# yewsiang/Transferable3D

Measured on AMD Instinct MI355X. Metric: frustums/sec fwd+bwd, higher is better.
Workload: dtype f32

## Files before the change

### include/t3d.h

```cpp
#ifndef T3D_H_
#define T3D_H_

#include <stdint.h>

#ifdef __cplusplus
extern "C" {
#endif

#define T3D_OK 0
#define T3D_ERR_ARG (-1)
#define T3D_ERR_SHAPE (-2)
#define T3D_ERR_LAUNCH (-3)
#define T3D_ERR_ABI (-4)

#define T3D_ABI_VERSION 3
#define T3D_V2_SIZE_pointmlp_fwd_args 200
#define T3D_V2_SIZE_pointmlp_dgrad_args 168
#define T3D_V2_SIZE_pointmlp_wgrad_args 144
#define T3D_V2_SIZE_pointmlp_dgrad_gram_args 168
#define T3D_V2_SIZE_pointmlp_gram_args 96
#define T3D_V2_SIZE_seg_head_args 208
#define T3D_V2_SIZE_boxpc_rep_args 104

#define T3D_TILE_ROWS 128
// ... 622 lines not shown
  int len;
  const int32_t* members;
  const int32_t* offsets;
  int n_groups;
} t3d_semi_list;
typedef struct {
  uint32_t struct_size;
  int method;
  t3d_semi_list list3d;
  t3d_semi_list list2d;
  const int32_t* perm;
  int perm_len;
  int B;
  uint32_t seed;
  float equal_prob;
  const float* hyper;
  int32_t* sample;
  int32_t* is_data_2D;
} t3d_semi_sample_args;
#define T3D_V2_SIZE_semi_sample_args 136
int t3d_semi_sample(const t3d_semi_sample_args* args, t3d_stream_t stream);

#define T3D_NUM_CLASS 10
typedef struct {
  uint32_t struct_size;
  int F;
  const int32_t* cls;
  const uint8_t* member;
  const int32_t* class_mask;
  float keep_prob;
  float add_prob;
  uint32_t seed;
  int reserved;
  int32_t* ids;
  int32_t* members;
  int32_t* offsets;
  int32_t* present;
  int32_t* summary;
} t3d_label_subset_args;
#define T3D_V2_SIZE_label_subset_args 88
int t3d_label_subset(const t3d_label_subset_args* args, t3d_stream_t stream);

typedef struct {
  float* center;
  int32_t* orient_cls;
  float* orient_reg;
  const int32_t* dims_cls;
  float* dims_reg;
  float* y_box_iou;
  float* y_center_delta;
  float* y_dims_delta;
  float* y_orient_delta;
  float center_perturbation, size_perturbation, angle_perturbation;
  float fit_lo, fit_hi, nofit_lo, nofit_hi, proportion_fit;
  const float* fit_draw;
  const float* cand_draws;
  int max_rounds;
  uint32_t seed;
  const float* hyper;
  int B;
} t3d_boxpc_perturb_args;
int t3d_boxpc_perturb(const t3d_boxpc_perturb_args* args, t3d_stream_t stream);


typedef struct { int64_t slab_off; int64_t grad_off; int32_t numel; int32_t n_slabs; } t3d_slab_desc;
int t3d_reduce_slabs(const float* slab_base, float* grad_base, const t3d_slab_desc* table_dev,
                     int n_tensors, int max_numel, t3d_stream_t stream);
int t3d_pool_bwd_mid(const float* slab_base, float* grad_base, const t3d_slab_desc* table_dev, int n_tensors, int max_numel,
                     const t3d_pool_sparse_rows_args* sparse, t3d_stream_t stream);

typedef struct {
  float base_lr, lr_decay_rate, lr_decay_step;
  float bn_init_decay, bn_decay_rate, bn_decay_step, bn_decay_clip;
  float beta1, beta2;
  int batch_size;
  int step_offset;
} t3d_schedule;
int t3d_schedule_step(float* hyper, const t3d_schedule* s, t3d_stream_t stream);

int t3d_adam_tf_step(float* params, const float* grads, float* m, float* v, int64_t n,
                     const float* hyper, float beta1, float beta2, float eps, float grad_scale,
                     t3d_stream_t stream);

int t3d_split_x3(const float* src, void* planes, int64_t n, int64_t plane_stride, t3d_stream_t stream);

typedef struct {
  int64_t off;
  int32_t K, N;
  int32_t fwd, dgrad;
  int32_t blk0;
  int32_t reserved;
} t3d_x3_frag_entry;
int t3d_split_x3_frag(const float* params, void* planes_fwd, void* planes_dgrad, int64_t plane_stride, const t3d_x3_frag_entry* table,
                      int n_entries, int n_blocks, t3d_stream_t stream);

int t3d_momentum_step(float* params, const float* grads, float* accum, int64_t n, const float* hyper, float momentum,
                      float grad_scale, t3d_stream_t stream);

typedef struct {
  t3d_act_src a;
  const float* mask;
  float keep_prob;
  float* out;
  int M, K;
  int rows_per_frustum;
} t3d_act_dropout_args;
int t3d_act_dropout(const t3d_act_dropout_args* args, t3d_stream_t stream);

int t3d_cast_bf16(const float* src, void* dst, int64_t n, t3d_stream_t stream);

int t3d_dropout_mask(float* mask, int64_t n, float keep_prob, uint32_t seed, const float* hyper,
                     t3d_stream_t stream);

enum { T3D_SMALL_BN_BWD_FINALIZE = 1, T3D_SMALL_FC_BWD = 2, T3D_SMALL_FC_DINPUT = 3, T3D_SMALL_DY_COLSUM = 4,
       T3D_SMALL_BN_FWD_FINALIZE = 5, T3D_SMALL_FC_FWD = 6, T3D_SMALL_POOL_BWD_MID = 7 };
typedef struct {
  const float* slab_base;
  float* grad_base;
  const t3d_slab_desc* table_dev;
  int n_tensors, max_numel;
  t3d_pool_sparse_rows_args sparse;
} t3d_pool_bwd_mid_args;
typedef struct {
  int kind;
  int depends;
  union {
    t3d_bn_bwd_finalize_args bn_bwd;
    t3d_fc_bwd_args fc_bwd;
    t3d_fc_dinput_args fc_dinput;
    t3d_dy_colsum_args dy_colsum;
    t3d_bn_fwd_finalize_args bn_fwd;
    t3d_fc_fwd_args fc_fwd;
    t3d_pool_bwd_mid_args mid;
  } u;
} t3d_small_op;
int t3d_small_pair(const t3d_small_op* a, const t3d_small_op* b, t3d_stream_t stream);

#define T3D_RIDER_MAX_OPS 10
typedef struct {
  t3d_small_op ops[T3D_RIDER_MAX_OPS];
  int n_ops;
  int n_wg;
  int lds_bytes;
  unsigned* sync;
} t3d_rider_set;
int t3d_riders_plan(t3d_rider_set* riders);
int t3d_run_riders(const t3d_rider_set* riders, t3d_stream_t stream);
int t3d_pointmlp_fwd_r(const t3d_pointmlp_fwd_args* args, const t3d_rider_set* riders, t3d_stream_t stream);
int t3d_pointmlp_wgrad_r(const t3d_pointmlp_wgrad_args* args, const t3d_rider_set* riders, t3d_stream_t stream);
int t3d_pointmlp_bwd_r(const t3d_pointmlp_dgrad_args* dgrad, const t3d_pointmlp_wgrad_args* wgrad, const t3d_rider_set* riders,
                       t3d_stream_t stream);
int t3d_pool_bwd_stage1_r(const t3d_pointmlp_gram_args* gram, const t3d_act_colsum_args* colsum, const t3d_pool_bwd_prep_args* prep,
                          const t3d_rider_set* riders, t3d_stream_t stream);
int t3d_pool_bwd_stage2_r(const t3d_pool_wgrad_finish_args* finish, const t3d_pointmlp_dgrad_gram_args* dgrad,
                          const t3d_rider_set* riders, t3d_stream_t stream);
int t3d_pointmlp_fwd_hosts_riders(const t3d_pointmlp_fwd_args* args);
int t3d_pointmlp_wgrad_hosts_riders(const t3d_pointmlp_wgrad_args* args);
int t3d_pointmlp_bwd_hosts_riders(const t3d_pointmlp_dgrad_args* dgrad, const t3d_pointmlp_wgrad_args* wgrad);
int t3d_pool_bwd_stage1_hosts_riders(const t3d_pointmlp_gram_args* gram, const t3d_act_colsum_args* colsum, const t3d_pool_bwd_prep_args* prep);
int t3d_pool_bwd_stage2_hosts_riders(const t3d_pool_wgrad_finish_args* finish, const t3d_pointmlp_dgrad_gram_args* dgrad);

typedef struct {
  uint32_t struct_size;
  const double* points;
  const int64_t* scene_offsets;
  const double* rtilt;
  const double* K;
  const int32_t* scene_jobs;
  int n_scenes; int max_scene_points; int C_src; int C; int n_jobs; int num_points;
  const double* box2d;
  int perturb_box2d;
  const double* perturb_draws;
  const double* box3d;
  const int32_t* job_key;
  uint32_t seed;
  const int32_t* choice;
  const int64_t* mask_offsets;
// ... 80 lines not shown
```

### transferable3d_amd/abi.py

```python
import ctypes as C
import os

F = C.POINTER(C.c_float)
I = C.POINTER(C.c_int32)
D = C.POINTER(C.c_double)
L = C.POINTER(C.c_int64)
i32, f32 = C.c_int, C.c_float

TILE_ROWS = 128
F32, BF16 = 0, 1
DTYPE_BY_NAME = {'f32': F32, 'bf16': BF16}
ARITH_AUTO, ARITH_FP32_MFMA, ARITH_BF16X3, ARITH_BF16 = 0, 1, 2, 3
ARITH_BY_NAME = {'auto': ARITH_AUTO, 'fp32_mfma': ARITH_FP32_MFMA, 'bf16x3': ARITH_BF16X3}
ARITH_NAMES = {ARITH_FP32_MFMA: 'fp32_mfma', ARITH_BF16X3: 'bf16x3', ARITH_BF16: 'bf16'}
ABI_VERSION = 3
ERR_ABI = -4
ACT_NONE, ACT_RELU, ACT_LEAKY_RELU, ACT_TANH = 0, 1, 2, 3
ACT_BY_NAME = {None: ACT_NONE, 'relu': ACT_RELU, 'leaky_relu': ACT_LEAKY_RELU, 'tanh': ACT_TANH}


class Sized(C.Structure):

    def __init__(self, *args, **kw):
        super().__init__(C.sizeof(type(self)), *args, **kw)
# ... 129 lines not shown
    _fields_ = [('in_', F), ('ld_in', i32), ('K', i32), ('in2', F), ('ld_in2', i32), ('K2', i32), ('w', F), ('bias', F),
                ('gamma', F), ('beta', F), ('moving_mean', F), ('moving_var', F), ('decay', F), ('eps', f32),
                ('is_training', i32), ('unbiased_ema', i32), ('act', i32), ('leaky_alpha', f32), ('drop_mask', F),
                ('keep_prob', f32), ('add_in', F), ('ld_add', i32), ('add_n', i32), ('y', F), ('out', F),
                ('ld_out', i32), ('mean', F), ('invstd', F), ('B', i32), ('N', i32)]


class FcBwdArgs(C.Structure):
    _fields_ = [('dout', F), ('ld_dout', i32), ('dy_next', F), ('w_next', F), ('N_next', i32),
                ('in_', F), ('ld_in', i32), ('K', i32), ('in2', F), ('ld_in2', i32), ('K2', i32),
                ('y', F), ('out', F), ('ld_out', i32), ('gamma', F), ('beta', F), ('mean', F), ('invstd', F),
                ('bn_training', i32), ('act', i32), ('leaky_alpha', f32), ('drop_mask', F), ('keep_prob', f32),
                ('dy', F), ('dw', F), ('dbias', F), ('dgamma', F), ('dbeta', F), ('B', i32), ('N', i32)]


class FcDinputArgs(C.Structure):
    _fields_ = [('dy', F), ('N', i32), ('w', F), ('add_in', F), ('ld_add', i32), ('alpha', f32), ('din', F),
                ('ld_din', i32), ('B', i32), ('K', i32),
                ('bn_pooled', F), ('bn_ld_pooled', i32), ('bn_ysel', F), ('bn_dpool', F), ('bn_count', i32), ('bn_gamma', F), ('bn_mean', F),
                ('bn_invstd', F), ('bn_scale', F), ('bn_frozen', i32), ('bn_dgamma', F), ('bn_dbeta', F), ('bn_coef', F)]


class SegHeadArgs(Sized):
    _fields_ = [('struct_size', C.c_uint32), ('y', F), ('scale', F), ('shift', F), ('drop_mask', F), ('keep_prob', f32), ('w', F), ('bias', F),
                ('labels', I), ('is_data_2D', I), ('pc', F), ('ld_pc', i32), ('ce_weight', f32), ('logits', F),
                ('mask', F), ('part', F), ('dz', F), ('psum_dz', F), ('psum_dzy', F), ('dw_part', F),
                ('M', i32), ('K', i32), ('rows_per_frustum', i32), ('B', i32), ('drop_seed', C.c_uint32), ('drop_hyper', F),
                ('dtype', i32), ('dsoft', F), ('oracle_mask', I)]


SMALL_KIND = {'t3d_bn_bwd_finalize': 1, 't3d_fc_bwd': 2, 't3d_fc_dinput': 3, 't3d_dy_colsum': 4}
RIDER_KIND = dict(SMALL_KIND, t3d_bn_fwd_finalize=5, t3d_fc_fwd=6, t3d_pool_bwd_mid=7)
RIDER_FIELD = {1: 'bn_bwd', 2: 'fc_bwd', 3: 'fc_dinput', 4: 'dy_colsum', 5: 'bn_fwd', 6: 'fc_fwd', 7: 'mid'}
RIDER_WIDE = ('t3d_pool_bwd_mid',)


class WeakLossArgs(C.Structure):
    _fields_ = [('center', F), ('reg_dims', F), ('reg_theta', F), ('pc', F), ('ld_pc', i32), ('logits', F), ('Rtilt', F), ('K', F),
                ('rot_frust', F), ('box2D', F), ('img_dim', F), ('is_data_2D', I), ('w_reproj', f32), ('w_surface', f32),
                ('multiplier', f32), ('use_softmax_proj', i32), ('softmax_scale', f32), ('dilate', f32), ('clip_lower_b_loss', i32),
                ('clip_pred_box', i32), ('loss_mse', i32), ('train_box_reproj', i32 * 3), ('train_box_surface', i32 * 3),
                ('surface_margin', f32), ('surface_scale_dims', f32), ('surf_part', F), ('dsoft', F), ('reproj', F), ('surface', F),
                ('dbox7', F), ('total_losses', F), ('loss', F), ('B', i32), ('N', i32), ('one_hot', F), ('w_inactive', f32),
                ('inactive_margins', f32 * 10), ('inactive_train', i32 * 10), ('inactive', F)]


class ActDropoutArgs(C.Structure):
    _fields_ = [('a', ActSrc), ('mask', F), ('keep_prob', f32), ('out', F), ('M', i32), ('K', i32), ('rows_per_frustum', i32)]


class SegFinalizeArgs(C.Structure):
    _fields_ = [('part', F), ('dw_part', F), ('B', i32), ('tiles_per_frustum', i32), ('rows_per_frustum', i32),
                ('K', i32), ('mask_xyz_mean', F), ('seg_loss', F), ('dw', F), ('dbias', F), ('n_correct', F)]


class StrongWeights(C.Structure):
    _fields_ = [(n, f32) for n in ('center', 'orient_cls', 'orient_reg', 'dims_cls', 'dims_reg', 'tnet_center',
                                   'corner', 'box_multiplier', 'cross_entropy')]


class StrongLossArgs(C.Structure):
    _fields_ = [('box', F), ('ld_box', i32), ('stage1_center', F), ('seg_loss', F), ('y_center', F),
                ('y_orient_cls', I), ('y_orient_reg', F), ('y_dims_cls', I), ('y_dims_reg', F), ('is_data_2D', I),
                ('wts', StrongWeights), ('normalize_by_3d_count', i32), ('dbox', F), ('dstage1', F), ('terms', F),
                ('total_losses', F), ('loss', F), ('center', F), ('reg_dims', F), ('reg_theta', F), ('iou2d', F), ('iou3d', F), ('B', i32)]


class X3FragEntry(C.Structure):
    _fields_ = [('off', C.c_int64), ('K', C.c_int32), ('N', C.c_int32), ('fwd', C.c_int32), ('dgrad', C.c_int32), ('blk0', C.c_int32), ('reserved', C.c_int32)]


def x3_frag_table(entries):
    import numpy as np
    rec = np.zeros(len(entries), dtype=np.dtype([('off', '<i8'), ('K', '<i4'), ('N', '<i4'), ('fwd', '<i4'), ('dgrad', '<i4'), ('blk0', '<i4'), ('reserved', '<i4')]))
    blk = 0
    for i, (off, K, N) in enumerate(entries):
        rec[i] = (off, K, N, 1, 1, blk, 0)
        blk += (K * N // 8 + 255) // 256
    return rec.view(np.uint8).copy(), blk


class SlabDesc(C.Structure):
    _fields_ = [('slab_off', C.c_int64), ('grad_off', C.c_int64), ('numel', C.c_int32), ('n_slabs', C.c_int32)]


class Schedule(C.Structure):
    _fields_ = [('base_lr', f32), ('lr_decay_rate', f32), ('lr_decay_step', f32), ('bn_init_decay', f32),
                ('bn_decay_rate', f32), ('bn_decay_step', f32), ('bn_decay_clip', f32), ('beta1', f32), ('beta2', f32),
                ('batch_size', i32), ('step_offset', i32)]


class BoxPcRepArgs(Sized):
    _fields_ = [('struct_size', C.c_uint32), ('pc', F), ('ld_pc', i32), ('C', i32), ('center', F), ('dims', F), ('theta', F), ('y_dims_cls', I),
                ('y_orient_cls', I), ('rep', F), ('ld_rep', i32), ('box_out', F), ('M', i32), ('rows_per_frustum', i32), ('rowmask', F)]


class BoxPcRepBArgs(C.Structure):
    _fields_ = [('center', F), ('dims', F), ('theta', F), ('y_dims_cls', I), ('y_orient_cls', I), ('box_out', F), ('pc', F), ('ld_pc', i32),
                ('C', i32), ('rowmask', F), ('pc_out', F), ('ld_out', i32), ('B', i32), ('rows_per_frustum', i32)]


class BoxPcRepBwdArgs(C.Structure):
    _fields_ = [('pc', F), ('ld_pc', i32), ('box', F), ('drep', F), ('ld_drep', i32), ('coff', i32), ('dbox', F),
                ('B', i32), ('rows_per_frustum', i32)]


class BoxPcLossArgs(C.Structure):
    _fields_ = [('out', F), ('y_box_iou', F), ('y_center_delta', F), ('y_dims_delta', F), ('y_orient_delta', F),
                ('fit_bound', f32), ('w_cls', f32), ('w_delta', f32), ('w_center', f32), ('w_size', f32), ('w_angle', f32),
                ('weigh_by_cls_conf', i32), ('weigh_by_cls_gt', i32), ('dout', F), ('terms', F), ('loss', F), ('B', i32),
                ('weigh_pred_by_cls_conf', i32), ('grad_cls_via_delta', i32), ('delta_loss_mse', i32)]


class BoxRefineStepBwdArgs(C.Structure):
    _fields_ = [('out9', F), ('dbox_rep', F), ('carry', F), ('tot_out', F), ('dout9', F), ('weigh_by_conf', i32),
                ('grad_via_conf', i32), ('B', i32)]


class Box2dFeatsArgs(C.Structure):
    _fields_ = [('one_hot', F), ('n_oh', i32), ('box2D', F), ('img_dim', F), ('out', F), ('B', i32)]


class DgradNarrowArgs(C.Structure):
    _fields_ = [('dy', DySrc), ('w', F), ('k0', i32), ('kn', i32), ('out', F), ('ld_out', i32), ('M', i32), ('N', i32)]


class SemiFinalLossArgs(C.Structure):
    _fields_ = [('strong_loss', F), ('reg_dims', F), ('one_hot', F), ('is_data_2D', I), ('out9', F),
                ('train_classes', C.c_int32 * 10), ('w_weak', f32), ('w_fit', f32), ('fit_only_2d', i32), ('d_dims', F),
                ('dout9', F), ('fit_prob', F), ('terms', F), ('loss', F), ('B', i32)]


class AnchorRegBwdArgs(C.Structure):
    _fields_ = [('box', F), ('ld_box', i32), ('dbox7', F), ('d_dims', F), ('dbox', F), ('dstage1', F), ('B', i32)]


class FrustumExtractArgs(Sized):
    _fields_ = [('struct_size', C.c_uint32), ('points', D), ('scene_offsets', L), ('rtilt', D), ('K', D), ('scene_jobs', I),
                ('n_scenes', i32), ('max_scene_points', i32), ('C_src', i32), ('C', i32), ('n_jobs', i32), ('num_points', i32),
                ('box2d', D), ('perturb_box2d', i32), ('perturb_draws', D), ('box3d', D), ('job_key', I), ('seed', C.c_uint32),
                ('choice', I), ('mask_offsets', L), ('masks', C.POINTER(C.c_uint64)), ('seg_prefix', I), ('box2d_out', D),
                ('frustum_angle', D), ('n_in_box', I), ('count', I), ('index', I), ('out_points', D), ('label', I)]


U8 = C.POINTER(C.c_uint8)


class SunrgbdEvalArgs(Sized):
    _fields_ = [('struct_size', C.c_uint32), ('P', i32), ('G', i32), ('det_centroid', D), ('det_basis', D), ('det_coeffs', D),
                ('det_confidence', D), ('det_image', I), ('gt_centroid', D), ('gt_basis', D), ('gt_coeffs', D), ('gt_image', I),
                ('gt_difficult', U8), ('n_images', i32), ('image_ids', I), ('image_gt_offsets', I), ('image_gt', I),
                ('threshold', C.c_double), ('workspace', C.c_void_p), ('workspace_bytes', C.c_uint64), ('order', I), ('max_overlap', D),
                ('gt_idx', I), ('is_tp', U8), ('is_fp', U8), ('gt_assignment', I), ('is_missed', U8), ('precision', D), ('recall', D),
                ('ap', D), ('overlap_offsets', L), ('overlaps', D), ('overlap_gt', I)]


SEMI_BATCH, SEMI_ALTERNATE_BATCH, SEMI_MIXED_BATCH = 0, 1, 2
SEMI_METHODS = {'BATCH': SEMI_BATCH, 'ALTERNATE_BATCH': SEMI_ALTERNATE_BATCH, 'MIXED_BATCH': SEMI_MIXED_BATCH}
SEMI_SAMPLE_MAX_B = 256


class SemiList(C.Structure):
    _fields_ = [('ids', I), ('len', i32), ('members', I), ('offsets', I), ('n_groups', i32)]


class SemiSampleArgs(Sized):
# ... 25 lines not shown
    _fields_ = [('slab_base', F), ('grad_base', F), ('table_dev', C.POINTER(SlabDesc)), ('n_tensors', i32), ('max_numel', i32),
                ('sparse', PoolSparseRowsArgs)]


class SmallOpU(C.Union):
    _fields_ = [('bn_bwd', BnBwdFinalizeArgs), ('fc_bwd', FcBwdArgs), ('fc_dinput', FcDinputArgs), ('dy_colsum', DyColsumArgs),
                ('bn_fwd', BnFwdFinalizeArgs), ('fc_fwd', FcFwdArgs), ('mid', PoolBwdMidArgs)]


class SmallOp(C.Structure):
    _fields_ = [('kind', i32), ('depends', i32), ('u', SmallOpU)]


RIDER_MAX_OPS = 10


class RiderSet(C.Structure):
    _fields_ = [('ops', SmallOp * RIDER_MAX_OPS), ('n_ops', i32), ('n_wg', i32), ('lds_bytes', i32), ('sync', C.POINTER(C.c_uint32))]


ENTRY_POINTS = {
    't3d_abi_version': [],
    't3d_gemm_arithmetic': [i32, i32, i32, i32, i32],
    't3d_source_hash': [C.c_char_p, C.c_int],
    't3d_pointmlp_fwd': [C.POINTER(PointMlpFwdArgs), VP],
    't3d_bn_fwd_finalize': [C.POINTER(BnFwdFinalizeArgs), VP],
    't3d_pool_finalize': [C.POINTER(PoolFinalizeArgs), VP],
    't3d_pointmlp_dgrad': [C.POINTER(PointMlpDgradArgs), VP],
    't3d_pointmlp_wgrad': [C.POINTER(PointMlpWgradArgs), VP],
    't3d_pointmlp_bwd': [C.POINTER(PointMlpDgradArgs), C.POINTER(PointMlpWgradArgs), VP],
    't3d_wgrad_plan': [i32, i32, i32, C.POINTER(i32), C.POINTER(i32), C.POINTER(i32)],
    't3d_bwd_plan': [i32, i32, i32, i32, C.POINTER(i32), C.POINTER(i32)],
    't3d_weak_loss': [C.POINTER(WeakLossArgs), VP],
    't3d_small_pair': [C.POINTER(SmallOp), C.POINTER(SmallOp), VP],
    't3d_riders_plan': [C.POINTER(RiderSet)],
    't3d_run_riders': [C.POINTER(RiderSet), VP],
    't3d_pointmlp_fwd_r': [C.POINTER(PointMlpFwdArgs), C.POINTER(RiderSet), VP],
    't3d_pointmlp_wgrad_r': [C.POINTER(PointMlpWgradArgs), C.POINTER(RiderSet), VP],
    't3d_pointmlp_bwd_r': [C.POINTER(PointMlpDgradArgs), C.POINTER(PointMlpWgradArgs), C.POINTER(RiderSet), VP],
    't3d_pool_bwd_stage1_r': [C.POINTER(PointMlpGramArgs), C.POINTER(ActColsumArgs), C.POINTER(PoolBwdPrepArgs), C.POINTER(RiderSet), VP],
    't3d_pool_bwd_stage2_r': [C.POINTER(PoolWgradFinishArgs), C.POINTER(PointMlpDgradGramArgs), C.POINTER(RiderSet), VP],
    't3d_pointmlp_fwd_hosts_riders': [C.POINTER(PointMlpFwdArgs)],
    't3d_pointmlp_wgrad_hosts_riders': [C.POINTER(PointMlpWgradArgs)],
    't3d_pointmlp_bwd_hosts_riders': [C.POINTER(PointMlpDgradArgs), C.POINTER(PointMlpWgradArgs)],
    't3d_pool_bwd_stage1_hosts_riders': [C.POINTER(PointMlpGramArgs), C.POINTER(ActColsumArgs), C.POINTER(PoolBwdPrepArgs)],
    't3d_pool_bwd_stage2_hosts_riders': [C.POINTER(PoolWgradFinishArgs), C.POINTER(PointMlpDgradGramArgs)],
    't3d_gram_plan': [i32, i32, i32, C.POINTER(i32), C.POINTER(i32)],
    't3d_bn_bwd_finalize': [C.POINTER(BnBwdFinalizeArgs), VP],
    't3d_dy_colsum': [C.POINTER(DyColsumArgs), VP],
    't3d_pool_bwd_prep': [C.POINTER(PoolBwdPrepArgs), VP],
    't3d_pool_sparse_rows': [C.POINTER(PoolSparseRowsArgs), VP],
    't3d_pointmlp_dgrad_gram': [C.POINTER(PointMlpDgradGramArgs), VP],
    't3d_pointmlp_gram': [C.POINTER(PointMlpGramArgs), VP],
    't3d_act_colsum': [C.POINTER(ActColsumArgs), VP],
    't3d_pool_wgrad_finish': [C.POINTER(PoolWgradFinishArgs), VP],
    't3d_batch_assemble': [C.POINTER(BatchAssembleArgs), VP],
    't3d_box_refine_step': [C.POINTER(BoxRefineStepArgs), VP],
    't3d_box_refine_step_bwd': [C.POINTER(BoxRefineStepBwdArgs), VP],
    't3d_boxpc_perturb': [C.POINTER(BoxPcPerturbArgs), VP],
    't3d_sample_equal_classes': [C.POINTER(SampleEqualClassesArgs), VP],
    't3d_box3d_iou': [C.POINTER(Box3dIouArgs), VP],
    't3d_box3d_iou_corners': [C.POINTER(Box3dIouCornersArgs), VP],
    't3d_box_head_iou': [C.POINTER(BoxHeadIouArgs), VP],
    't3d_box2d_feats': [C.POINTER(Box2dFeatsArgs), VP],
    't3d_pool_bwd_stage1': [C.POINTER(PointMlpGramArgs), C.POINTER(ActColsumArgs), C.POINTER(PoolBwdPrepArgs), VP],
    't3d_pool_bwd_mid': [F, F, C.POINTER(SlabDesc), i32, i32, C.POINTER(PoolSparseRowsArgs), VP],
    't3d_pool_bwd_stage2': [C.POINTER(PoolWgradFinishArgs), C.POINTER(PointMlpDgradGramArgs), VP],
    't3d_fc_fwd': [C.POINTER(FcFwdArgs), VP],
    't3d_fc_bwd': [C.POINTER(FcBwdArgs), VP],
    't3d_fc_dinput': [C.POINTER(FcDinputArgs), VP],
    't3d_seg_head': [C.POINTER(SegHeadArgs), VP],
    't3d_seg_finalize': [C.POINTER(SegFinalizeArgs), VP],
    't3d_act_dropout': [C.POINTER(ActDropoutArgs), VP],
    't3d_strong_loss': [C.POINTER(StrongLossArgs), VP],
    't3d_boxpc_rep': [C.POINTER(BoxPcRepArgs), VP],
    't3d_boxpc_rep_b': [C.POINTER(BoxPcRepBArgs), VP],
    't3d_boxpc_rep_bwd': [C.POINTER(BoxPcRepBwdArgs), VP],
    't3d_boxpc_loss': [C.POINTER(BoxPcLossArgs), VP],
    't3d_pointmlp_dgrad_narrow': [C.POINTER(DgradNarrowArgs), VP],
    't3d_semi_final_loss': [C.POINTER(SemiFinalLossArgs), VP],
    't3d_anchor_reg_bwd': [C.POINTER(AnchorRegBwdArgs), VP],
    't3d_reduce_slabs': [F, F, C.POINTER(SlabDesc), i32, i32, VP],
    't3d_schedule_step': [F, C.POINTER(Schedule), VP],
    't3d_adam_tf_step': [F, F, F, F, C.c_int64, F, f32, f32, f32, f32, VP],
    't3d_momentum_step': [F, F, F, C.c_int64, F, f32, f32, VP],
    't3d_split_x3': [F, VP, C.c_int64, C.c_int64, VP],
    't3d_split_x3_frag': [F, VP, VP, C.c_int64, VP, i32, i32, VP],
    't3d_dropout_mask': [F, C.c_int64, f32, C.c_uint32, F, VP],
    't3d_cast_bf16': [F, VP, C.c_int64, VP],
    't3d_frustum_extract': [C.POINTER(FrustumExtractArgs), VP],
    't3d_sunrgbd_eval': [C.POINTER(SunrgbdEvalArgs), VP],
    't3d_detect_decode': [C.POINTER(DetectDecodeArgs), VP],
    't3d_semi_sample': [C.POINTER(SemiSampleArgs), VP],
    't3d_label_subset': [C.POINTER(LabelSubsetArgs), VP],
}

LIB_PATH = os.path.join(os.path.dirname(os.path.abspath(__file__)), 'libt3d.so')
ERRORS = {-1: 'T3D_ERR_ARG', -2: 'T3D_ERR_SHAPE', -3: 'T3D_ERR_LAUNCH'}


class T3DError(RuntimeError):
    pass


def source_hash_of(lib):
    buf = C.create_string_buffer(64)
    check(lib.t3d_source_hash(buf, 64), 't3d_source_hash')
    return buf.value.decode()


def load(path=None):
    import torch
    variant = path or os.environ.get('T3D_LIB')
    path = variant or LIB_PATH
    if not os.path.exists(path):
        raise T3DError('HIP library %s not built: run `python -m transferable3d_amd.build` (no CPU fallback exists)' % path)
    lib = C.CDLL(path)
    for name, argtypes in ENTRY_POINTS.items():
        fn = getattr(lib, name, None)
        if fn is None:
            raise T3DError('%s does not export %s' % (path, name))
        fn.argtypes = argtypes
        fn.restype = C.c_int
    if lib.t3d_abi_version() != ABI_VERSION:
        raise T3DError('%s speaks ABI version %d, this host side version %d (include/t3d.h): rebuild it' % (path, lib.t3d_abi_version(), ABI_VERSION))
    from .build import CSRC, lib_source_hash
    if not variant and os.path.isdir(CSRC) and os.environ.get('T3D_ALLOW_STALE_LIB', '0') != '1':
        built, src = source_hash_of(lib), lib_source_hash()
        if built != src:
            raise T3DError('%s was built from other sources (library %s, csrc/ + include/t3d.h %s): run '
                           '`python -m transferable3d_amd.build`' % (path, built, src))
    return lib


def fptr(t):
    return C.cast(C.c_void_p(0 if t is None else t.data_ptr()), F)


def iptr(t):
    return C.cast(C.c_void_p(0 if t is None else t.data_ptr()), I)


def u8ptr(t):
    return C.cast(C.c_void_p(0 if t is None else t.data_ptr()), U8)


def check(rc, what):
    if rc != 0:
        raise T3DError('%s failed: %s' % (what, ERRORS.get(rc, rc)))
```

### transferable3d_amd/csrc/bn_dev.h

```cpp
#pragma once
#include "common.h"
#include <math.h>

namespace {

constexpr int FC_CH = 16, FC_GR = 16, FC_GR_BIG = 64, FC_CH_WIDE = 4, FC_GR_WIDE = 256, FC_WIDE_MAX_N = 128;

template <int NQ, int GR = FC_GR, int U = 16>
__device__ __forceinline__ void tile_sums(const float* const (&src)[NQ], int n_tiles, int N, int c, int grp, bool ok,
                                          double (&acc)[NQ]) {
#pragma unroll
  for (int q = 0; q < NQ; ++q) acc[q] = 0.0;
  if (!ok) return;
  for (int t0 = grp; t0 < n_tiles; t0 += U * GR) {
    float v[NQ][U];
#pragma unroll
    for (int q = 0; q < NQ; ++q)
#pragma unroll
      for (int u = 0; u < U; ++u) {
        const int t = t0 + u * GR;
        const float x = src[q][(size_t)min(t, n_tiles - 1) * N + c];
        v[q][u] = t < n_tiles ? x : 0.f;
      }
#pragma unroll
// ... 98 lines not shown
      const bool take = (t0 + u < tiles_per_frustum) && a[u] >= 0 && (arg < 0 || (use_max ? v[u] > best : v[u] < best));
      best = take ? v[u] : best;
      arg = take ? a[u] : arg;
    }
  }
  float out = 0.f;
  if (arg >= 0) out = fmaxf(fmaf(best, sc, sh), 0.f);
  const bool live = out > 0.f;
  const size_t i = (size_t)b * N + c;
  pooled[(size_t)b * ld_pooled + c] = out;
  argidx[i] = live ? arg : -1;
  ysel[i] = live ? best : 0.f;
}
__device__ __forceinline__ void pool_pick(const t3d_bn_fwd_finalize_args& p, int b, int c, float sc, float sh) {
  pool_pick_impl(p.pool_pmax, p.pool_pmin, p.pool_pamax, p.pool_pamin, p.pool_tiles_per_frustum, p.N, b, c, sc, sh, p.pooled,
                 p.ld_pooled, p.argidx, p.ysel);
}

template <int GR, int CH = FC_CH>
__device__ __forceinline__ void bn_fwd_finalize_body(const t3d_bn_fwd_finalize_args& p, double (*red)[CH], float* s_scsh, const int bid) {
  const int cl = threadIdx.x & (CH - 1), grp = threadIdx.x / CH;
  const int c = bid * CH + cl;
  const bool ok = c < p.N;
  if (p.is_training) {
    const int cc = ok ? c : 0;
    const float gam = p.gamma[cc], bet = p.beta[cc], mm = p.moving_mean[cc], mv = p.moving_var[cc], dec = p.decay[0];
    const float* const src[2] = {p.psum, p.psumsq};
    double acc[2];
    tile_sums<2, GR, (GR > 64 ? 8 : 16)>(src, p.n_tiles, p.N, c, grp, ok, acc);
    const double s = group_reduce<GR, CH>(acc[0], red, grp, cl);
    const double ss = group_reduce<GR, CH>(acc[1], red, grp, cl);
    if (grp == 0 && ok) {
      const double n = (double)p.count;
      const double mean = s / n;
      double var = ss / n - mean * mean;
      if (var < 0.0) var = 0.0;
      const double invstd = 1.0 / sqrt(var + (double)p.eps);
      const double sc = (double)gam * invstd;
      p.scale[c] = (float)sc;
      p.shift[c] = (float)((double)bet - mean * sc);
      p.mean[c] = (float)mean;
      p.invstd[c] = (float)invstd;
      const double d = (double)dec;
      const double var_ema = p.unbiased_ema ? var * (n / (n > 1.0 ? n - 1.0 : 1.0)) : var;
      p.moving_mean[c] = (float)((double)mm * d + mean * (1.0 - d));
      p.moving_var[c] = (float)((double)mv * d + var_ema * (1.0 - d));
    }
  } else if (grp == 0 && ok) {
    const double invstd = 1.0 / sqrt((double)p.moving_var[c] + (double)p.eps);
    const double sc = (double)p.gamma[c] * invstd;
    p.scale[c] = (float)sc;
    p.shift[c] = (float)((double)p.beta[c] - (double)p.moving_mean[c] * sc);
    p.mean[c] = p.moving_mean[c];
    p.invstd[c] = (float)invstd;
  }
  if (p.pool_pmax != nullptr) {
    float* s_sc = s_scsh;
    float* s_sh = s_scsh + CH;
    __syncthreads();
    if (grp == 0 && ok) { s_sc[cl] = p.scale[c]; s_sh[cl] = p.shift[c]; }
    __syncthreads();
    if (ok) {
      const float sc = s_sc[cl], sh = s_sh[cl];
      for (int b = grp; b < p.pool_B; b += GR) pool_pick(p, b, c, sc, sh);
    }
  }
}

__device__ __forceinline__ void dy_colsum_body(const t3d_dy_colsum_args& p, const int bid, const int tid) {
  const int i = bid * 256 + tid;
  if (tid >= 256 || i >= p.B * p.N) return;
  const int b = i / p.N, c = i % p.N;
  double sdz = 0.0, sy = 0.0;
  for (int t = 0; t < p.tiles_per_frustum; ++t) {
    const size_t o = (size_t)(b * p.tiles_per_frustum + t) * p.N + c;
    sdz += (double)p.psum_dz[o];
    sy += (double)p.psum_y[o];
  }
  const double v = (double)p.coef[c] * sdz + (double)p.coef[p.N + c] * sy +
                   (double)p.coef[2 * p.N + c] * (double)p.rows_per_frustum;
  p.out[i] = (float)((double)p.alpha * v);
}

__device__ __forceinline__ void reduce_slabs_body(const float* __restrict__ slab_base, float* __restrict__ grad_base,
                                                  const t3d_slab_desc* __restrict__ table, float4 (*part)[32], int bx, int by,
                                                  int gx) {
  const t3d_slab_desc d = table[by];
  const bool vec = ((d.slab_off | d.grad_off | (int64_t)d.numel) & 3) == 0;
  const int n4 = vec ? (d.numel >> 2) : 0;
  const int el = threadIdx.x & 31, grp = threadIdx.x >> 5;
  for (int e0 = bx * 32; e0 < n4; e0 += gx * 32) {
    const int e = e0 + el;
    float4 a0 = make_float4(0.f, 0.f, 0.f, 0.f), a1 = a0, a2 = a0, a3 = a0;
    if (e < n4) {
      const float4* s = reinterpret_cast<const float4*>(slab_base + d.slab_off) + e;
      int k = grp;
      for (; k + 56 < d.n_slabs; k += 64) {
        float4 v[8];
#pragma unroll
        for (int u = 0; u < 8; ++u) v[u] = s[(size_t)(k + 8 * u) * n4];
#pragma unroll
        for (int u = 0; u < 8; u += 4) {
          a0.x += v[u].x; a0.y += v[u].y; a0.z += v[u].z; a0.w += v[u].w;
          a1.x += v[u + 1].x; a1.y += v[u + 1].y; a1.z += v[u + 1].z; a1.w += v[u + 1].w;
          a2.x += v[u + 2].x; a2.y += v[u + 2].y; a2.z += v[u + 2].z; a2.w += v[u + 2].w;
          a3.x += v[u + 3].x; a3.y += v[u + 3].y; a3.z += v[u + 3].z; a3.w += v[u + 3].w;
        }
      }
      for (; k + 24 < d.n_slabs; k += 32) {
        const float4 v0 = s[(size_t)(k + 0) * n4], v1 = s[(size_t)(k + 8) * n4], v2 = s[(size_t)(k + 16) * n4],
                     v3 = s[(size_t)(k + 24) * n4];
        a0.x += v0.x; a0.y += v0.y; a0.z += v0.z; a0.w += v0.w;
        a1.x += v1.x; a1.y += v1.y; a1.z += v1.z; a1.w += v1.w;
        a2.x += v2.x; a2.y += v2.y; a2.z += v2.z; a2.w += v2.w;
        a3.x += v3.x; a3.y += v3.y; a3.z += v3.z; a3.w += v3.w;
      }
      for (; k < d.n_slabs; k += 8) {
        const float4 v = s[(size_t)k * n4];
        a0.x += v.x; a0.y += v.y; a0.z += v.z; a0.w += v.w;
      }
    }
    float4 r;
    r.x = (a0.x + a1.x) + (a2.x + a3.x); r.y = (a0.y + a1.y) + (a2.y + a3.y);
    r.z = (a0.z + a1.z) + (a2.z + a3.z); r.w = (a0.w + a1.w) + (a2.w + a3.w);
    part[grp][el] = r;
    __syncthreads();
    if (grp == 0 && e < n4) {
      float4 t = part[0][el];
#pragma unroll
      for (int g = 1; g < 8; ++g) {
        const float4 u = part[g][el];
        t.x += u.x; t.y += u.y; t.z += u.z; t.w += u.w;
      }
      reinterpret_cast<float4*>(grad_base + d.grad_off)[e] = t;
    }
    __syncthreads();
  }
  if (!vec) {
    for (int e = bx * blockDim.x + threadIdx.x; e < d.numel; e += gx * blockDim.x) {
      float acc = 0.f;
      for (int k = 0; k < d.n_slabs; ++k) acc += slab_base[d.slab_off + (size_t)k * d.numel + e];
      grad_base[d.grad_off + e] = acc;
    }
  }
}


}
```

### transferable3d_amd/csrc/bn_optim.hip

```cpp
#include "common.h"
#include "poolbwd_dev.h"
#include "bn_dev.h"

namespace {

template <int GR, int CH = FC_CH>
__global__ __launch_bounds__(GR * CH) void k_bn_fwd_finalize(const t3d_bn_fwd_finalize_args p) {
  __shared__ double red[GR][CH];
  __shared__ float s_scsh[2 * CH];
  bn_fwd_finalize_body<GR, CH>(p, red, s_scsh, blockIdx.x);
}

__global__ __launch_bounds__(256) void k_pool_finalize(const t3d_pool_finalize_args p) {
  const int i = blockIdx.x * blockDim.x + threadIdx.x;
  if (i >= p.B * p.N) return;
  const int b = i / p.N, c = i % p.N;
  pool_pick_impl(p.pmax, p.pmin, p.pamax, p.pamin, p.tiles_per_frustum, p.N, b, c, p.scale[c], p.shift[c], p.pooled, p.ld_pooled,
                 p.argidx, p.ysel);
}

template <int GR, int CH = FC_CH>
__global__ __launch_bounds__(GR * CH) void k_bn_bwd_finalize(const t3d_bn_bwd_finalize_args p) {
  __shared__ double red[GR][CH];
  bn_bwd_finalize_body<GR, CH>(p, red, blockIdx.x, threadIdx.x);
}

__global__ __launch_bounds__(256) void k_dy_colsum(const t3d_dy_colsum_args p) { dy_colsum_body(p, blockIdx.x, threadIdx.x); }

__global__ __launch_bounds__(256) void k_reduce_slabs(const float* __restrict__ slab_base, float* __restrict__ grad_base,
                                                      const t3d_slab_desc* __restrict__ table) {
  __shared__ float4 part[8][32];
  reduce_slabs_body(slab_base, grad_base, table, part, blockIdx.x, blockIdx.y, gridDim.x);
}

__global__ __launch_bounds__(256) void k_pool_bwd_mid(const float* __restrict__ slab_base, float* __restrict__ grad_base,
                                                      const t3d_slab_desc* __restrict__ table, const int gx, const int n_reduce,
                                                      const t3d_pool_sparse_rows_args sp) {
  extern __shared__ __attribute__((aligned(16))) float smem[];
  const int b = blockIdx.x;
  if (b < n_reduce) {
    reduce_slabs_body(slab_base, grad_base, table, reinterpret_cast<float4(*)[32]>(smem), b % gx, b / gx, gx);
  } else {
    const int r = b - n_reduce, tiles = sp.B * sp.rows_per_frustum / 128;
    pool_sparse_rows_body(sp, smem, r % tiles, r / tiles);
  }
}

__global__ __launch_bounds__(64) void k_schedule_step(float* hyper, const t3d_schedule s) {
  if (blockIdx.x != 0) return;
  const int lane = threadIdx.x;
  const double step = (double)hyper[0] + (double)s.step_offset;
  const double seen = step * (double)s.batch_size;
  const double t = step + 1.0;
  const double base = lane == 0 ? (double)s.lr_decay_rate : lane == 1 ? (double)s.bn_decay_rate : lane == 2 ? (double)s.beta2 : (double)s.beta1;
  const double expo = lane == 0 ? floor(seen / (double)s.lr_decay_step) : lane == 1 ? floor(seen / (double)s.bn_decay_step) : t;
  const double pw = lane < 4 ? pow(base, expo) : 0.0;
  const double p_lr = __shfl(pw, 0), p_bn = __shfl(pw, 1), p_b2 = __shfl(pw, 2), p_b1 = __shfl(pw, 3);
  if (lane != 0) return;
  const double lr = (double)s.base_lr * p_lr;
  const double bnm = (double)s.bn_init_decay * p_bn;
  const double bnd = fmin((double)s.bn_decay_clip, 1.0 - bnm);
  const double lr_t = lr * sqrt(1.0 - p_b2) / (1.0 - p_b1);
  hyper[1] = (float)lr;
  hyper[2] = (float)bnd;
  hyper[3] = (float)lr_t;
  hyper[0] = (float)t;
}

__global__ __launch_bounds__(256) void k_adam_tf(float* __restrict__ w, const float* __restrict__ g, float* __restrict__ m,
                                                 float* __restrict__ v, int64_t n, const float* __restrict__ hyper,
                                                 float b1, float b2, float eps, float gscale) {
  const float lr_t = hyper[3];
  for (int64_t i = (int64_t)blockIdx.x * blockDim.x + threadIdx.x; i < n; i += (int64_t)gridDim.x * blockDim.x) {
    const float gi = g[i] * gscale;
    const float mi = b1 * m[i] + (1.f - b1) * gi;
    const float vi = b2 * v[i] + (1.f - b2) * gi * gi;
    m[i] = mi;
    v[i] = vi;
    w[i] -= lr_t * mi / (sqrtf(vi) + eps);
  }
}

__global__ __launch_bounds__(256) void k_momentum_tf(float* __restrict__ w, const float* __restrict__ g, float* __restrict__ acc,
                                                     int64_t n, const float* __restrict__ hyper, float momentum, float gscale) {
  const float lr = hyper[1];
  for (int64_t i = (int64_t)blockIdx.x * blockDim.x + threadIdx.x; i < n; i += (int64_t)gridDim.x * blockDim.x) {
    const float a = fmaf(momentum, acc[i], g[i] * gscale);
    acc[i] = a;
    w[i] -= lr * a;
  }
}

__device__ __forceinline__ uint32_t mix_u32(uint64_t x) {
  x ^= x >> 33; x *= 0xff51afd7ed558ccdULL;
  x ^= x >> 33; x *= 0xc4ceb9fe1a85ec53ULL;
  x ^= x >> 33;
  return (uint32_t)(x >> 16);
}
__global__ __launch_bounds__(256) void k_dropout_mask(float* __restrict__ mask, int64_t n, float keep, uint32_t seed,
                                                      const float* __restrict__ hyper) {
  const uint64_t step = (uint64_t)hyper[0];
  const uint64_t key = ((uint64_t)seed << 32) ^ (step * 0x9E3779B97F4A7C15ULL);
  for (int64_t i = (int64_t)blockIdx.x * blockDim.x + threadIdx.x; i < n; i += (int64_t)gridDim.x * blockDim.x) {
    const uint32_t r = mix_u32(key + (uint64_t)i * 0xD6E8FEB86659FD93ULL);
    const float u = (float)(r >> 8) * (1.0f / 16777216.0f);
    mask[i] = u < keep ? 1.f : 0.f;
  }
}

}

extern "C" int t3d_abi_version(void) { return T3D_ABI_VERSION; }

static int fin_big_tiles() {
  static const int v = []() { const char* e = getenv("T3D_FIN_BIG"); const int x = e ? atoi(e) : 512; return x > 0 ? x : (1 << 30); }();
  return v;
}

static int fin_wide_tiles() {
  static const int v = []() { const char* e = getenv("T3D_FIN_WIDE"); const int x = e ? atoi(e) : 1024; return x > 0 ? x : (1 << 30); }();
  return v;
}

extern "C" int t3d_bn_fwd_finalize(const t3d_bn_fwd_finalize_args* a, t3d_stream_t stream) {
  if (!a || !a->gamma || !a->beta || !a->moving_mean || !a->moving_var || !a->scale || !a->shift || !a->mean ||
      !a->invstd)
    return T3D_ERR_ARG;
  if (a->is_training && (!a->psum || !a->psumsq || !a->decay || a->count <= 0)) return T3D_ERR_ARG;
  if (a->is_training && a->n_tiles >= fin_wide_tiles() && a->N <= FC_WIDE_MAX_N)
    T3D_LAUNCH((k_bn_fwd_finalize<FC_GR_WIDE, FC_CH_WIDE>), dim3((a->N + FC_CH_WIDE - 1) / FC_CH_WIDE), dim3(FC_GR_WIDE * FC_CH_WIDE), 0,
               static_cast<hipStream_t>(stream), *a);
  else if (a->is_training && a->n_tiles > fin_big_tiles())
    T3D_LAUNCH(k_bn_fwd_finalize<FC_GR_BIG>, dim3((a->N + FC_CH - 1) / FC_CH), dim3(FC_GR_BIG * FC_CH), 0, static_cast<hipStream_t>(stream), *a);
  else
    T3D_LAUNCH(k_bn_fwd_finalize<FC_GR>, dim3((a->N + FC_CH - 1) / FC_CH), dim3(FC_GR * FC_CH), 0, static_cast<hipStream_t>(stream), *a);
  T3D_CHECK_LAUNCH();
  return T3D_OK;
}

extern "C" int t3d_pool_finalize(const t3d_pool_finalize_args* a, t3d_stream_t stream) {
  if (!a || !a->scale || !a->shift || !a->pmax || !a->pmin || !a->pamax || !a->pamin || !a->pooled || !a->argidx ||
      !a->ysel)
    return T3D_ERR_ARG;
  T3D_LAUNCH(k_pool_finalize, dim3((a->B * a->N + 255) / 256), dim3(256), 0, static_cast<hipStream_t>(stream),
                     *a);
  T3D_CHECK_LAUNCH();
  return T3D_OK;
}

extern "C" int t3d_bn_bwd_finalize(const t3d_bn_bwd_finalize_args* a, t3d_stream_t stream) {
  if (!a || !a->coef) return T3D_ERR_ARG;
  if (a->psum_dz == nullptr && (!a->dpool_in || !a->pooled || !a->ysel || !a->dpool)) return T3D_ERR_ARG;
  if (a->psum_dz != nullptr && !a->psum_dzy) return T3D_ERR_ARG;
  if (a->frozen ? !a->scale : (!a->gamma || !a->mean || !a->invstd)) return T3D_ERR_ARG;
  if (a->psum_dz != nullptr && a->n_tiles >= fin_wide_tiles() && a->N <= FC_WIDE_MAX_N)
    T3D_LAUNCH((k_bn_bwd_finalize<FC_GR_WIDE, FC_CH_WIDE>), dim3((a->N + FC_CH_WIDE - 1) / FC_CH_WIDE), dim3(FC_GR_WIDE * FC_CH_WIDE), 0,
               static_cast<hipStream_t>(stream), *a);
  else if (a->psum_dz != nullptr && a->n_tiles > fin_big_tiles())
    T3D_LAUNCH(k_bn_bwd_finalize<FC_GR_BIG>, dim3((a->N + FC_CH - 1) / FC_CH), dim3(FC_GR_BIG * FC_CH), 0, static_cast<hipStream_t>(stream), *a);
  else
    T3D_LAUNCH(k_bn_bwd_finalize<FC_GR>, dim3((a->N + FC_CH - 1) / FC_CH), dim3(FC_GR * FC_CH), 0, static_cast<hipStream_t>(stream), *a);
  T3D_CHECK_LAUNCH();
  return T3D_OK;
}

extern "C" int t3d_dy_colsum(const t3d_dy_colsum_args* a, t3d_stream_t stream) {
  if (!a || !a->psum_dz || !a->psum_y || !a->coef || !a->out) return T3D_ERR_ARG;
  T3D_LAUNCH(k_dy_colsum, dim3((a->B * a->N + 255) / 256), dim3(256), 0, static_cast<hipStream_t>(stream), *a);
  T3D_CHECK_LAUNCH();
  return T3D_OK;
}

extern "C" int t3d_reduce_slabs(const float* slab_base, float* grad_base, const t3d_slab_desc* table_dev, int n_tensors,
                                int max_numel, t3d_stream_t stream) {
  if (!slab_base || !grad_base || !table_dev || n_tensors <= 0) return T3D_ERR_ARG;
  int gx = (max_numel / 4 + 31) / 32;
  if (gx > 256) gx = 256;
  if (gx < 1) gx = 1;
  T3D_LAUNCH(k_reduce_slabs, dim3(gx, n_tensors), dim3(256), 0, static_cast<hipStream_t>(stream), slab_base,
                     grad_base, table_dev);
  T3D_CHECK_LAUNCH();
  return T3D_OK;
}

extern "C" int t3d_schedule_step(float* hyper, const t3d_schedule* s, t3d_stream_t stream) {
  if (!hyper || !s) return T3D_ERR_ARG;
  T3D_LAUNCH(k_schedule_step, dim3(1), dim3(64), 0, static_cast<hipStream_t>(stream), hyper, *s);
  T3D_CHECK_LAUNCH();
  return T3D_OK;
}

extern "C" int t3d_adam_tf_step(float* params, const float* grads, float* m, float* v, int64_t n, const float* hyper,
                                float beta1, float beta2, float eps, float grad_scale, t3d_stream_t stream) {
  if (!params || !grads || !m || !v || !hyper || n <= 0) return T3D_ERR_ARG;
  int64_t blocks = (n + 255) / 256;
  if (blocks > 2048) blocks = 2048;
  T3D_LAUNCH(k_adam_tf, dim3((unsigned)blocks), dim3(256), 0, static_cast<hipStream_t>(stream), params, grads, m,
                     v, n, hyper, beta1, beta2, eps, grad_scale);
  T3D_CHECK_LAUNCH();
  return T3D_OK;
}

extern "C" int t3d_momentum_step(float* params, const float* grads, float* accum, int64_t n, const float* hyper, float momentum,
                                 float grad_scale, t3d_stream_t stream) {
  if (!params || !grads || !accum || !hyper || n <= 0) return T3D_ERR_ARG;
  int64_t blocks = (n + 255) / 256;
  if (blocks > 2048) blocks = 2048;
  T3D_LAUNCH(k_momentum_tf, dim3((unsigned)blocks), dim3(256), 0, static_cast<hipStream_t>(stream), params, grads, accum, n, hyper,
             momentum, grad_scale);
  T3D_CHECK_LAUNCH();
  return T3D_OK;
}

__global__ __launch_bounds__(256) void k_cast_bf16(const float* __restrict__ src, bf16_t* __restrict__ dst, int64_t n) {
  const int64_t stride = (int64_t)gridDim.x * 256 * 8;
  for (int64_t i = ((int64_t)blockIdx.x * 256 + threadIdx.x) * 8; i < n; i += stride) {
    if (i + 8 <= n) {
      const float4 a = *reinterpret_cast<const float4*>(src + i), b = *reinterpret_cast<const float4*>(src + i + 4);
      const bf16x8 h = {(bf16_t)a.x, (bf16_t)a.y, (bf16_t)a.z, (bf16_t)a.w, (bf16_t)b.x, (bf16_t)b.y, (bf16_t)b.z, (bf16_t)b.w};
      *reinterpret_cast<bf16x8*>(dst + i) = h;
    } else {
      for (int64_t j = i; j < n; ++j) dst[j] = (bf16_t)src[j];
    }
  }
}

extern "C" int t3d_cast_bf16(const float* src, void* dst, int64_t n, t3d_stream_t stream) {
  if (!src || !dst || n <= 0 || (reinterpret_cast<uintptr_t>(src) & 15) || (reinterpret_cast<uintptr_t>(dst) & 15)) return T3D_ERR_ARG;
  int64_t blocks = (n + 2047) / 2048;
  if (blocks > 2048) blocks = 2048;
  T3D_LAUNCH(k_cast_bf16, dim3((unsigned)blocks), dim3(256), 0, static_cast<hipStream_t>(stream), src, static_cast<bf16_t*>(dst), n);
  T3D_CHECK_LAUNCH();
  return T3D_OK;
}

extern "C" int t3d_dropout_mask(float* mask, int64_t n, float keep_prob, uint32_t seed, const float* hyper,
                                t3d_stream_t stream) {
  if (!mask || !hyper || n <= 0) return T3D_ERR_ARG;
  int64_t blocks = (n + 255) / 256;
  if (blocks > 4096) blocks = 4096;
  T3D_LAUNCH(k_dropout_mask, dim3((unsigned)blocks), dim3(256), 0, static_cast<hipStream_t>(stream), mask, n,
                     keep_prob, seed, hyper);
  T3D_CHECK_LAUNCH();
  return T3D_OK;
}

extern "C" int t3d_pool_bwd_mid(const float* slab_base, float* grad_base, const t3d_slab_desc* table_dev, int n_tensors,
                                int max_numel, const t3d_pool_sparse_rows_args* a, t3d_stream_t stream) {
  if (!slab_base || !grad_base || !table_dev || n_tensors <= 0) return T3D_ERR_ARG;
  const int rc = check_sparse_rows(a);
  if (rc != T3D_OK) return rc;
  int gx = (max_numel / 4 + 31) / 32;
  if (gx > 256) gx = 256;
  if (gx < 1) gx = 1;
  const int n_reduce = gx * n_tensors;
  const long M = (long)a->B * a->rows_per_frustum;
  const int n_sparse = (int)(M / 128) * (a->K / SR_KC);
  const size_t lds = sparse_rows_lds(a->N);
  static size_t allowed = 0;
  if (lds > 64 * 1024 && lds > allowed) {
    (void)hipFuncSetAttribute(reinterpret_cast<const void*>(k_pool_bwd_mid), hipFuncAttributeMaxDynamicSharedMemorySize, (int)lds);
    allowed = lds;
  }
  T3D_LAUNCH(k_pool_bwd_mid, dim3(n_reduce + n_sparse), dim3(256), lds, static_cast<hipStream_t>(stream), slab_base, grad_base,
             table_dev, gx, n_reduce, *a);
  T3D_CHECK_LAUNCH();
  return T3D_OK;
}
```

### transferable3d_amd/csrc/pointmlp.hip

```cpp
#include "common.h"
#include "poolbwd_dev.h"
#include "rider_dev.h"

#include <cstdlib>
#include <mutex>
#include <type_traits>
#include <utility>
#include <unordered_map>

namespace {

constexpr int BK = 32;
constexpr int MIN_WAVES_PER_EU = 2;
constexpr int LDR = BK + 4;
constexpr int NT = 256;

__device__ __forceinline__ float4 f4zero() { return make_float4(0.f, 0.f, 0.f, 0.f); }

__device__ __forceinline__ unsigned keep_bits32(const float* __restrict__ rowmask, int base) {
  float4 m[8];
#pragma unroll
  for (int q = 0; q < 8; ++q) m[q] = *reinterpret_cast<const float4*>(rowmask + base + (q >> 2) * 32 + (q & 3) * 8);
  unsigned bits = 0u;
#pragma unroll
// ... 1675 lines not shown
          for (int r = 0; r < 16; ++r) {
            const float v = SY ? Elem<bf16_t>::rnd(acc[tm][tn][r] + add) : acc[tm][tn][r] + add;
            if constexpr (SY) ytile[(wm * 64 + 4 * h + tm * 32 + (r & 3) + 8 * (r >> 2)) * YLD + wn * (BN / 2) + tn * 32 + l31] = (bf16_t)v;
            s_ += v;
            ss = fmaf(v, v, ss);
            if constexpr (PL) {
              const bool keep = (keepbits >> (tm * 16 + r)) & 1u;
              const int rin = rin_base + tm * 32 + (r & 3) + 8 * (r >> 2);
              const bool up = keep & (v > mx), dn = keep & (v < mn);
              mx = up ? v : mx;
              ax = up ? rin : ax;
              mn = dn ? v : mn;
              an = dn ? rin : an;
            }
          }
        }
        s_ += __shfl_xor(s_, 32, 64);
        ss += __shfl_xor(ss, 32, 64);
        if constexpr (PL) {
          const float omx = __shfl_xor(mx, 32, 64), omn = __shfl_xor(mn, 32, 64);
          const int oax = __shfl_xor(ax, 32, 64), oan = __shfl_xor(an, 32, 64);
          if (oax >= 0 && (omx > mx || ax < 0 || (omx == mx && oax < ax))) { mx = omx; ax = oax; }
          if (oan >= 0 && (omn < mn || an < 0 || (omn == mn && oan < an))) { mn = omn; an = oan; }
        }
        csum[tn] = s_; csq[tn] = ss; cmax[tn] = mx; cmin[tn] = mn; amax[tn] = ax; amin[tn] = an;
      }
    };
    if (store_y) { if (pool) epi(std::true_type{}, std::true_type{}); else epi(std::true_type{}, std::false_type{}); }
    else { if (pool) epi(std::false_type{}, std::true_type{}); else epi(std::false_type{}, std::false_type{}); }
    if (h == 0) {
#pragma unroll
      for (int tn = 0; tn < TN; ++tn) {
        const int c = wn * (BN / 2) + tn * 32 + l31;
        red[(0 * 2 + wm) * BN + c] = csum[tn];
        red[(1 * 2 + wm) * BN + c] = csq[tn];
        if (pool) {
          red[(2 * 2 + wm) * BN + c] = cmax[tn];
          red[(3 * 2 + wm) * BN + c] = cmin[tn];
          reinterpret_cast<int*>(red)[(4 * 2 + wm) * BN + c] = amax[tn];
          reinterpret_cast<int*>(red)[(5 * 2 + wm) * BN + c] = amin[tn];
        }
      }
    }
    if (tr_first && nt == 0) T3D_TRACE_MARK8(4);
    __syncthreads();
    if (tid < BN) {
      const int c = tid;
      const size_t o = (size_t)tile_m * p.N + col0 + c;
      p.psum[o] = red[(0 * 2 + 0) * BN + c] + red[(0 * 2 + 1) * BN + c];
      p.psumsq[o] = red[(1 * 2 + 0) * BN + c] + red[(1 * 2 + 1) * BN + c];
      if (pool) {
        float mx = red[(2 * 2 + 0) * BN + c], mn = red[(3 * 2 + 0) * BN + c];
        int ax = reinterpret_cast<int*>(red)[(4 * 2 + 0) * BN + c], an = reinterpret_cast<int*>(red)[(5 * 2 + 0) * BN + c];
        const float mx1 = red[(2 * 2 + 1) * BN + c], mn1 = red[(3 * 2 + 1) * BN + c];
        const int ax1 = reinterpret_cast<int*>(red)[(4 * 2 + 1) * BN + c], an1 = reinterpret_cast<int*>(red)[(5 * 2 + 1) * BN + c];
        if (ax1 >= 0 && (ax < 0 || mx1 > mx)) { mx = mx1; ax = ax1; }
        if (an1 >= 0 && (an < 0 || mn1 < mn)) { mn = mn1; an = an1; }
        p.pmax[o] = mx; p.pmin[o] = mn; p.pamax[o] = ax; p.pamin[o] = an;
      }
    }
    if (tr_first && nt == 0) T3D_TRACE_MARK8(5);
    if constexpr (LAST) {
      fetch_w0(0, (tile_nx * 128) / p.rows_per_frustum);
      if constexpr (PREF) fetch_panel_coefs();
    } else {
      fetch_w0(col0 + BN, b);
    }
    if (store_y) {
#pragma unroll
      for (int i = 0; i < 128 * CPR / NT; ++i) {
        const int c = tid + NT * i, row = c / CPR, ch = c % CPR;
        *reinterpret_cast<bf16x8*>(yg + (size_t)(row0 + row) * p.N + col0 + ch * 8) = *reinterpret_cast<const bf16x8*>(ytile + row * YLD + ch * 8);
      }
    }
    if (tr_first && nt == 0) T3D_TRACE_MARK8(6);
  };
#pragma unroll 1
  for (int nt = 0; nt < n_tiles - 1; ++nt) col_tile(nt, std::false_type{});
  col_tile(n_tiles - 1, std::true_type{});
 }
  T3D_TRACE_MARK8(7);
}

template <int N, class YT = bf16_t>
__global__ __launch_bounds__(NT) void k_pointmlp_fwd_tinyk(const t3d_pointmlp_fwd_args p) {
  constexpr bool H = Elem<YT>::BF16;
  constexpr int CPR = N / 8, RPP = NT / CPR, NP = 128 / RPP;
  __shared__ float red[2][RPP][N];
  const int tid = threadIdx.x, ch = tid % CPR, r0 = tid / CPR;
  const int tile = blockIdx.x, row0 = tile * 128, b = row0 / p.rows_per_frustum;
  float w[4][8], add[8];
#pragma unroll
  for (int k = 0; k < 4; ++k) {
    if (H) {
      const bf16x8 v = *reinterpret_cast<const bf16x8*>(reinterpret_cast<const bf16_t*>(p.w) + (size_t)min(k, p.K - 1) * p.N + ch * 8);
#pragma unroll
      for (int e = 0; e < 8; ++e) w[k][e] = k < p.K ? (float)v[e] : 0.f;
    } else {
      const float4 v0 = *reinterpret_cast<const float4*>(p.w + (size_t)min(k, p.K - 1) * p.N + ch * 8);
      const float4 v1 = *reinterpret_cast<const float4*>(p.w + (size_t)min(k, p.K - 1) * p.N + ch * 8 + 4);
      const float v[8] = {v0.x, v0.y, v0.z, v0.w, v1.x, v1.y, v1.z, v1.w};
#pragma unroll
      for (int e = 0; e < 8; ++e) w[k][e] = k < p.K ? v[e] : 0.f;
    }
  }
#pragma unroll
  for (int e = 0; e < 8; ++e) add[e] = p.bias ? p.bias[ch * 8 + e] : 0.f;
  float sc[4] = {1.f, 1.f, 1.f, 1.f}, sh[4] = {0.f, 0.f, 0.f, 0.f}, sub[4] = {0.f, 0.f, 0.f, 0.f};
  if (p.a.scale != nullptr) {
    const float4 a = *reinterpret_cast<const float4*>(p.a.scale), c = *reinterpret_cast<const float4*>(p.a.shift);
    sc[0] = a.x; sc[1] = a.y; sc[2] = a.z; sc[3] = a.w; sh[0] = c.x; sh[1] = c.y; sh[2] = c.z; sh[3] = c.w;
  }
  if (p.a.sub != nullptr) {
#pragma unroll
    for (int k = 0; k < 4; ++k) sub[k] = p.a.sub[(size_t)b * p.a.sub_ld + min(k, p.K - 1)];
  }
  const float floor_ = p.a.relu ? 0.f : -INFINITY;
  float s1[8], s2[8];
#pragma unroll
  for (int e = 0; e < 8; ++e) { s1[e] = 0.f; s2[e] = 0.f; }
  float4 xs[NP];
#pragma unroll
  for (int i = 0; i < NP; ++i) xs[i] = *reinterpret_cast<const float4*>(p.a.x + (size_t)(row0 + r0 + RPP * i) * p.a.ldx + p.a.coff);
#pragma unroll
  for (int i = 0; i < NP; ++i) {
    const float xv[4] = {xs[i].x, xs[i].y, xs[i].z, xs[i].w};
    float a[4];
#pragma unroll
    for (int k = 0; k < 4; ++k) {
      const float t = fmaxf(fmaf(xv[k], sc[k], sh[k]), floor_) - sub[k];
      a[k] = k < p.K ? Elem<YT>::rnd(t) : 0.f;
    }
    float o[8];
#pragma unroll
    for (int e = 0; e < 8; ++e) {
      float acc = a[0] * w[0][e];
      acc = fmaf(a[1], w[1][e], acc);
      acc = fmaf(a[2], w[2][e], acc);
      acc = fmaf(a[3], w[3][e], acc);
      const float v = Elem<YT>::rnd(acc + add[e]);
      o[e] = v;
      s1[e] += v;
      s2[e] = fmaf(v, v, s2[e]);
    }
    const size_t off = (size_t)(row0 + r0 + RPP * i) * p.N + ch * 8;
    if (H) {
      bf16x8 ob;
#pragma unroll
      for (int e = 0; e < 8; ++e) ob[e] = (bf16_t)o[e];
      *reinterpret_cast<bf16x8*>(reinterpret_cast<bf16_t*>(p.y) + off) = ob;
    } else {
      *reinterpret_cast<float4*>(p.y + off) = make_float4(o[0], o[1], o[2], o[3]);
      *reinterpret_cast<float4*>(p.y + off + 4) = make_float4(o[4], o[5], o[6], o[7]);
    }
  }
#pragma unroll
  for (int e = 0; e < 8; ++e) { red[0][r0][ch * 8 + e] = s1[e]; red[1][r0][ch * 8 + e] = s2[e]; }
  __syncthreads();
  if (tid < N) {
    float t1 = 0.f, t2 = 0.f;
#pragma unroll
    for (int r = 0; r < RPP; ++r) { t1 += red[0][r][tid]; t2 += red[1][r][tid]; }
    p.psum[(size_t)tile * p.N + tid] = t1;
    p.psumsq[(size_t)tile * p.N + tid] = t2;
  }
}

struct DgradEpilogue {
  const float* add_in;
  const int32_t* add_live;
  const float* colconst;
  const float* prev_y;
  const float* prev_scale;
  const float* prev_shift;
  float* out;
  float* psum_dz;
  float* psum_dzy;
  int K;
};

template <int BN, int TM, int TN, int ADD, bool MASK>
__device__ __forceinline__ void dgrad_epilogue_body(const DgradEpilogue& p, f32x16 (&acc)[TM][TN], float* red, int tid,
                                                    int row0, int col0, int tile_m) {
  const int lane = tid & 63, wid = tid >> 6, wm = wid >> 1, wn = wid & 1;
  const int l31 = lane & 31, h = lane >> 5;
  const bool stats = MASK && p.psum_dz != nullptr;
  const unsigned K = (unsigned)p.K;
  float cs1[TN], cs2[TN];
  unsigned live = 0u;
  if (ADD == 2) {
    int4 fl[TM][4];
#pragma unroll
    for (int tm = 0; tm < TM; ++tm)
#pragma unroll
      for (int j = 0; j < 4; ++j) fl[tm][j] = *reinterpret_cast<const int4*>(p.add_live + row0 + wm * 64 + 4 * h + tm * 32 + 8 * j);
#pragma unroll
    for (int tm = 0; tm < TM; ++tm)
#pragma unroll
      for (int j = 0; j < 4; ++j) {
        const int4 f = fl[tm][j];
        live |= (unsigned)((f.x != 0) | ((f.y != 0) << 1) | ((f.z != 0) << 2) | ((f.w != 0) << 3)) << (tm * 16 + 4 * j);
      }
  }
#pragma unroll
  for (int tn = 0; tn < TN; ++tn) {
    const int col = col0 + wn * (BN / 2) + tn * 32 + l31;
    const float psc = MASK ? p.prev_scale[col] : 0.f, psh = MASK ? p.prev_shift[col] : 0.f;
    const float cc = p.colconst ? p.colconst[col] : 0.f;
    unsigned boff0 = ((unsigned)(row0 + wm * 64 + 4 * h) * K + (unsigned)col) * 4u;
    asm volatile("" : "+v"(boff0));
    const unsigned k4 = K * 4u;
    const char* const pyb = reinterpret_cast<const char*>(p.prev_y);
    const char* const adb = reinterpret_cast<const char*>(p.add_in);
    char* const outb = reinterpret_cast<char*>(p.out);
    float s1 = 0.f, s2 = 0.f;
#pragma unroll
    for (int tm = 0; tm < TM; ++tm) {
      constexpr int EB = 8;
#pragma unroll
      for (int r0 = 0; r0 < 16; r0 += EB) {
        float yp[EB], ad[EB];
#pragma unroll
        for (int e = 0; e < EB; ++e) {
          const int r = r0 + e;
          const unsigned o = boff0 + (unsigned)(tm * 32 + (r & 3) + 8 * (r >> 2)) * k4;
          yp[e] = MASK ? *reinterpret_cast<const float*>(pyb + o) : 0.f;
          if (ADD == 2) ad[e] = ((live >> (tm * 16 + r)) & 1u) ? *reinterpret_cast<const float*>(adb + o) : 0.f;
          else ad[e] = ADD ? *reinterpret_cast<const float*>(adb + o) : 0.f;
        }
#pragma unroll
        for (int e = 0; e < EB; ++e) {
          const int r = r0 + e;
          const unsigned o = boff0 + (unsigned)(tm * 32 + (r & 3) + 8 * (r >> 2)) * k4;
          float v = acc[tm][tn][r] + cc + ad[e];
          if (MASK) {
            if (!(fmaf(yp[e], psc, psh) > 0.f)) v = 0.f;
            s1 += v;
            s2 = fmaf(v, yp[e], s2);
          }
          *reinterpret_cast<float*>(outb + o) = v;
        }
      }
    }
    s1 += __shfl_xor(s1, 32, 64);
    s2 += __shfl_xor(s2, 32, 64);
    cs1[tn] = s1; cs2[tn] = s2;
  }
  if (stats) {
// ... 1460 lines not shown
  static std::unordered_map<const void*, size_t> done;
  std::lock_guard<std::mutex> lock(mu);
  size_t& cur = done[kernel];
  if (cur >= lds_bytes) return;
  (void)hipFuncSetAttribute(kernel, hipFuncAttributeMaxDynamicSharedMemorySize, (int)lds_bytes);
  cur = lds_bytes;
}

template <class Args>
void launch_lds(void (*kernel)(const Args), dim3 grid, size_t lds_bytes, hipStream_t s, const Args& a) {
  allow_lds(reinterpret_cast<const void*>(kernel), lds_bytes);
  T3D_LAUNCH(kernel, grid, dim3(NT), lds_bytes, s, a);
}
template <class Args>
void launch_lds_r(void (*kernel)(const Args, const t3d_rider_set), dim3 grid, size_t lds_bytes, hipStream_t s, const Args& a,
                  const t3d_rider_set& r) {
  allow_lds(reinterpret_cast<const void*>(kernel), lds_bytes);
  T3D_LAUNCH(kernel, grid, dim3(NT), lds_bytes, s, a, r);
}
template <class Args>
void launch_lds1(void (*kernel)(const Args), dim3 grid, size_t lds_bytes, hipStream_t s, const Args& a) {
  allow_lds(reinterpret_cast<const void*>(kernel), lds_bytes);
  T3D_LAUNCH(kernel, grid, dim3(NT1), lds_bytes, s, a);
}
constexpr size_t lds_fwd(int bn) { return 2 * (size_t)(128 * LDR + BK * bn) * sizeof(float); }
constexpr size_t lds_dgrad(int bn) { return 2 * (size_t)(128 * LDR + bn * LDR) * sizeof(float); }
constexpr size_t lds_wgrad(int bmk, int bn) { return 2 * (size_t)BK * (bmk + bn) * sizeof(float); }
constexpr size_t lds_epi(int bn) { return (size_t)12 * bn * sizeof(float) + (size_t)128 * (bn + 8) * 2; }
constexpr size_t lds_min(size_t b, int bn) { return b > lds_epi(bn) ? b : lds_epi(bn); }
constexpr size_t lds_fwd_h(int bn) { return lds_min(2 * (size_t)(128 * LDRH + BKH * (bn + 32)) * 2, bn); }
constexpr size_t lds_dgram_h(int bn) { return lds_fwd_h(bn) > (size_t)12 * bn * 4 + 2 * (size_t)128 * (bn + 8) * 2 ? lds_fwd_h(bn) : (size_t)12 * bn * 4 + 2 * (size_t)128 * (bn + 8) * 2; }
constexpr size_t lds_epi2(int bn) { return (size_t)12 * bn * sizeof(float) + 2 * (size_t)128 * (bn + 8) * 2; }
constexpr size_t lds_max(size_t a, size_t b) { return a > b ? a : b; }
constexpr size_t lds_dgrad_h(int bn) { return lds_max(2 * (size_t)(128 * LDRH + bn * LDRH) * 2, lds_epi2(bn)); }
constexpr size_t lds_wgrad_h(int bmk, int bn) { return 2 * (size_t)BKH * (bmk + 32 + bn + 32) * 2; }
constexpr size_t lds_x3_r(int dim) { return (size_t)3 * dim * LDRX * 2; }
constexpr size_t lds_x3_c(int dim) { return (size_t)3 * BKX * (dim + LDCX_PAD) * 2; }
constexpr size_t lds_fwd_x3(int bn) { return lds_max(2 * (lds_x3_r(128) + lds_x3_c(bn)), (size_t)12 * bn * sizeof(float)); }
constexpr size_t lds_dgrad_x3(int bn) { return lds_max(2 * (lds_x3_r(128) + lds_x3_r(bn)), (size_t)12 * bn * sizeof(float)); }
constexpr size_t lds_wgrad_x3(int bmk, int bn) { return 2 * (lds_x3_c(bmk) + lds_x3_c(bn)); }
constexpr size_t lds_bwd1f(int k, int n) { return (size_t)(64 * ((n + 4) + 3 * (k + 4)) + 2 * 2 * 2 * k + 3 * n + 2 * k) * 4; }
constexpr size_t lds_bwd1(int k, int n, int bm) { return (size_t)bm * (n + k + 2 * (k + 8)) * 2 + (size_t)2 * 2 * 4 * k * 4; }

bool dtype_ok(int dt) { return dt == T3D_F32 || dt == T3D_BF16; }
bool x3_on(int arith) {
  if (arith == T3D_ARITH_FP32_MFMA) return false;
  if (arith == T3D_ARITH_BF16X3) return true;
  const char* e = getenv("T3D_X3");
  return e ? atoi(e) != 0 : true;
}
long x3_min_kn(int arith) { const char* e = arith == T3D_ARITH_AUTO ? getenv("T3D_X3_MINKN") : nullptr; return e ? atol(e) : 1L; }
long x3_min_kn_bwd(int arith) { const char* e = arith == T3D_ARITH_AUTO ? getenv("T3D_X3_MINKN_BWD") : nullptr; return e ? atol(e) : x3_min_kn(arith); }
bool x3_layer(int arith, int K, int N) { return x3_on(arith) && (long)K * N >= x3_min_kn(arith) && K <= 4096 && N <= 4096; }
bool x3_bwd_narrow() { const char* e = getenv("T3D_X3_BWD_NARROW"); return e ? atoi(e) != 0 : true; }
bool x3_layer_bwd(int arith, int K, int N) {
  return x3_on(arith) && (long)K * N >= x3_min_kn_bwd(arith) && (N <= 4 * K || K >= 128 || x3_bwd_narrow()) && K <= 4096 && N <= 4096;
}
bool act_ok(const t3d_act_src& a, int K) {
  return a.x != nullptr && (a.ldx % 4) == 0 && (a.coff % 4) == 0 && a.coff + (K + 3) / 4 * 4 <= a.ldx &&
         (a.scale == nullptr || a.shift != nullptr) && dtype_ok(a.dtype) && !(a.dtype == T3D_BF16 && a.sub != nullptr) &&
         !(a.dtype == T3D_BF16 && ((a.ldx | a.coff) & 7));
}
bool dy_ok(const t3d_dy_src& d) {
  return d.y != nullptr && d.coef != nullptr && (d.dz != nullptr || (d.argidx != nullptr && d.dpool != nullptr)) && dtype_ok(d.dtype) &&
         !(d.dtype == T3D_BF16 && d.dz == nullptr);
}

bool riders_ok(const t3d_rider_set* r) {
  return r->sync != nullptr && r->n_ops > 0 && r->n_ops <= T3D_RIDER_MAX_OPS && r->n_wg > 0 && r->n_wg <= (r->n_ops == 1 ? RIDER_MAX_WG_WIDE : RIDER_MAX_WG) && r->lds_bytes >= 0;
}
size_t lds_with(size_t lds, const t3d_rider_set* r) { return r && (size_t)r->lds_bytes > lds ? (size_t)r->lds_bytes : lds; }

}

int t3d_x3_fwd(const t3d_pointmlp_fwd_args* a, const t3d_rider_set* r, hipStream_t s);
int t3d_x3_bwd(const t3d_pointmlp_dgrad_args* d, const t3d_pointmlp_wgrad_args* w, const t3d_rider_set* r, int tk, int tn, bool wide,
               int n_w, int n_d, hipStream_t s);
int t3d_x3_stage1(const t3d_pointmlp_gram_args* g, const t3d_act_colsum_args* c, const t3d_pool_bwd_prep_args* q, const t3d_rider_set* r,
                  int gt, int n_gram, int n_colsum, int n_prep, size_t lds_other, hipStream_t s);
int t3d_x3_stage2(const t3d_pool_wgrad_finish_args* f, const t3d_pointmlp_dgrad_gram_args* d, const t3d_rider_set* r, bool wide,
                  int n_finish, int n_d, size_t lds_other, hipStream_t s);
int t3d_x3_split(const float* src, void* planes, int64_t n, int64_t plane_stride, hipStream_t s);
int t3d_x3_split_frag(const float* params, void* pf, void* pd, int64_t stride, const t3d_x3_frag_entry* tab, int n, int n_blocks, hipStream_t s);
int t3d_x3_dgrad(const t3d_pointmlp_dgrad_args* a, bool wide, hipStream_t s);
int t3d_x3_wgrad(const t3d_pointmlp_wgrad_args* a, int tk, int tn, int n_blocks, hipStream_t s);
int t3d_x3_gram(const t3d_pointmlp_gram_args* a, int tk, int n_blocks, hipStream_t s);
int t3d_x3_dgrad_gram(const t3d_pointmlp_dgrad_gram_args* a, bool wide, hipStream_t s);

#ifdef T3D_X3_TU
namespace {
__global__ __launch_bounds__(256) void k_split_x3(const float* __restrict__ src, bf16_t* __restrict__ planes, long n, long stride) {
  const long step = (long)gridDim.x * 256 * 4;
  for (long i = ((long)blockIdx.x * 256 + threadIdx.x) * 4; i < n; i += step) {
    if (i + 4 <= n) {
      bf16x4 h, m, l;
      split3(*reinterpret_cast<const float4*>(src + i), h, m, l);
      *reinterpret_cast<bf16x4*>(planes + i) = h;
      *reinterpret_cast<bf16x4*>(planes + stride + i) = m;
      *reinterpret_cast<bf16x4*>(planes + 2 * stride + i) = l;
    } else {
      for (long j = i; j < n; ++j) {
        bf16x4 h, m, l;
        split3(make_float4(src[j], 0.f, 0.f, 0.f), h, m, l);
        planes[j] = h[0]; planes[stride + j] = m[0]; planes[2 * stride + j] = l[0];
      }
    }
  }
}
}
namespace {
__global__ __launch_bounds__(256) void k_split_x3_frag(const float* __restrict__ params, bf16_t* __restrict__ pf, bf16_t* __restrict__ pd, long stride,
                                                       const t3d_x3_frag_entry* __restrict__ tab, int n) {
  int e = 0;
  while (e + 1 < n && (int)blockIdx.x >= tab[e + 1].blk0) ++e;
  const t3d_x3_frag_entry en = tab[e];
  const float* w = params + en.off;
  const long nfr = (long)en.K * en.N / 8;
  const long f = (long)((int)blockIdx.x - en.blk0) * 256 + threadIdx.x;
  if (f >= nfr) return;
  const int lane = (int)(f & 63);
  const long q = f >> 6;
  float4 v0, v1, u0, u1;
  if (en.fwd) {
    const int NB = en.N / 32, nb = (int)(q % NB);
    const long k0 = (q / NB) * 16 + 8 * (lane >> 5);
    const float* src = w + k0 * en.N + nb * 32 + (lane & 31);
    v0 = make_float4(src[0], src[en.N], src[2 * (long)en.N], src[3 * (long)en.N]);
    v1 = make_float4(src[4 * (long)en.N], src[5 * (long)en.N], src[6 * (long)en.N], src[7 * (long)en.N]);
  }
  if (en.dgrad) {
    const int KB = en.K / 32, kb = (int)(q % KB);
    const long n0 = (q / KB) * 16 + 8 * (lane >> 5);
    const float* src = w + (long)(kb * 32 + (lane & 31)) * en.N + n0;
    u0 = *reinterpret_cast<const float4*>(src);
    u1 = *reinterpret_cast<const float4*>(src + 4);
  }
  bf16x4 h0, m0, l0, h1, m1, l1;
  if (en.fwd) {
    split3(v0, h0, m0, l0);
    split3(v1, h1, m1, l1);
    bf16_t* d = pf + en.off + f * 8;
    *reinterpret_cast<bf16x8*>(d) = __builtin_shufflevector(h0, h1, 0, 1, 2, 3, 4, 5, 6, 7);
    *reinterpret_cast<bf16x8*>(d + stride) = __builtin_shufflevector(m0, m1, 0, 1, 2, 3, 4, 5, 6, 7);
    *reinterpret_cast<bf16x8*>(d + 2 * stride) = __builtin_shufflevector(l0, l1, 0, 1, 2, 3, 4, 5, 6, 7);
  }
  if (en.dgrad) {
    split3(u0, h0, m0, l0);
    split3(u1, h1, m1, l1);
    bf16_t* d = pd + en.off + f * 8;
    *reinterpret_cast<bf16x8*>(d) = __builtin_shufflevector(h0, h1, 0, 1, 2, 3, 4, 5, 6, 7);
    *reinterpret_cast<bf16x8*>(d + stride) = __builtin_shufflevector(m0, m1, 0, 1, 2, 3, 4, 5, 6, 7);
    *reinterpret_cast<bf16x8*>(d + 2 * stride) = __builtin_shufflevector(l0, l1, 0, 1, 2, 3, 4, 5, 6, 7);
  }
}
}
int t3d_x3_split_frag(const float* params, void* pf, void* pd, int64_t stride, const t3d_x3_frag_entry* tab, int n, int n_blocks, hipStream_t s) {
  T3D_LAUNCH(k_split_x3_frag, dim3(n_blocks), dim3(256), 0, s, params, static_cast<bf16_t*>(pf), static_cast<bf16_t*>(pd), (long)stride, tab, n);
  T3D_CHECK_LAUNCH();
  return T3D_OK;
}
int t3d_x3_split(const float* src, void* planes, int64_t n, int64_t plane_stride, hipStream_t s) {
  long blocks = (n + 1023) / 1024;
  if (blocks > 2048) blocks = 2048;
  T3D_LAUNCH(k_split_x3, dim3((unsigned)blocks), dim3(256), 0, s, src, static_cast<bf16_t*>(planes), (long)n, (long)plane_stride);
  T3D_CHECK_LAUNCH();
  return T3D_OK;
}

int t3d_x3_dgrad(const t3d_pointmlp_dgrad_args* a, bool wide, hipStream_t s) {
  const int tiles_m = a->M / 128;
  if (a->w_x3 && (a->K % 32 != 0 || a->N % 16 != 0 || a->w_x3_stride < (int64_t)a->K * a->N)) return T3D_ERR_SHAPE;
  if (a->w_x3 && a->N <= X3_CTAB_MAX_CH) {
    if (wide) launch_lds(k_pointmlp_dgrad<128, false, PathX3P>, dim3(tiles_m * (a->K / 128)), lds_dgrad_x3(128), s, *a);
    else launch_lds(k_pointmlp_dgrad<64, false, PathX3P>, dim3(tiles_m * (a->K / 64)), lds_dgrad_x3(64), s, *a);
  } else if (wide) launch_lds(k_pointmlp_dgrad<128, false, PathX3>, dim3(tiles_m * (a->K / 128)), lds_dgrad_x3(128), s, *a);
  else launch_lds(k_pointmlp_dgrad<64, false, PathX3>, dim3(tiles_m * (a->K / 64)), lds_dgrad_x3(64), s, *a);
  T3D_CHECK_LAUNCH();
  return T3D_OK;
}

int t3d_x3_wgrad(const t3d_pointmlp_wgrad_args* a, int tk, int tn, int n_blocks, hipStream_t s) {
  const dim3 grid(n_blocks);
#define T3D_WGX(TK, TN_) launch_lds(k_pointmlp_wgrad<TK, TN_, false, false, PathX3, float>, grid, lds_wgrad_x3(TK, TN_), s, *a)
  if (tk == 128 && tn == 128) T3D_WGX(128, 128);
  else if (tk == 128) T3D_WGX(128, 64);
  else if (tn == 128) T3D_WGX(64, 128);
  else T3D_WGX(64, 64);
#undef T3D_WGX
  T3D_CHECK_LAUNCH();
  return T3D_OK;
}

int t3d_x3_gram(const t3d_pointmlp_gram_args* a, int tk, int n_blocks, hipStream_t s) {
  if (tk != 64) return T3D_ERR_ARG;
  launch_lds(k_pointmlp_gram<64, 64, PathX3>, dim3(n_blocks), lds_wgrad_x3(64, 64), s, *a);
  T3D_CHECK_LAUNCH();
  return T3D_OK;
}

int t3d_x3_dgrad_gram(const t3d_pointmlp_dgrad_gram_args* a, bool wide, hipStream_t s) {
  const int tiles_m = a->M / 128;
  if (wide) launch_lds(k_pointmlp_dgrad_gram<128, PathX3>, dim3(tiles_m * (a->K / 128)), lds_fwd_x3(128), s, *a);
  else launch_lds(k_pointmlp_dgrad_gram<64, PathX3>, dim3(tiles_m * (a->K / 64)), lds_fwd_x3(64), s, *a);
  T3D_CHECK_LAUNCH();
  return T3D_OK;
}

int t3d_x3_fwd(const t3d_pointmlp_fwd_args* a, const t3d_rider_set* r, hipStream_t s) {
  const int tiles_m = a->M / 128, nr = r ? r->n_wg : 0;
  const bool pre = a->w_x3 != nullptr && a->K <= X3_CTAB_MAX_CH;
  if (pre && (a->N % 32 != 0 || a->K % 16 != 0 || a->w_x3_stride < (int64_t)a->K * a->N)) return T3D_ERR_SHAPE;
  const int w8 = []() { const char* e_ = getenv("T3D_X3_W8"); return e_ ? atoi(e_) : 1; }();
  if (w8 && a->N % 256 == 0 && (w8 == 2 || (long)tiles_m * (a->N / 256) >= 512)) {
    const int n_tiles = tiles_m * (a->N / 256);
    const dim3 grid((n_tiles > T3D_FAIR_CUS ? T3D_FAIR_CUS : n_tiles) + nr);
    const size_t lds = lds_with(lds_fwd_x3(256), r);
    if (r && pre) {
      auto kern = k_pointmlp_fwd_w8_r<256, PathX3WP>;
      allow_lds(reinterpret_cast<const void*>(kern), lds);
      T3D_LAUNCH(kern, grid, dim3(2 * NT), lds, s, *a, *r, n_tiles);
    } else if (r) {
      auto kern = k_pointmlp_fwd_w8_r<256, PathX3W>;
      allow_lds(reinterpret_cast<const void*>(kern), lds);
      T3D_LAUNCH(kern, grid, dim3(2 * NT), lds, s, *a, *r, n_tiles);
    } else if (pre) {
      auto kern = k_pointmlp_fwd_w8<256, PathX3WP>;
      allow_lds(reinterpret_cast<const void*>(kern), lds);
      T3D_LAUNCH(kern, grid, dim3(2 * NT), lds, s, *a, n_tiles);
    } else {
      auto kern = k_pointmlp_fwd_w8<256, PathX3W>;
      allow_lds(reinterpret_cast<const void*>(kern), lds);
      T3D_LAUNCH(kern, grid, dim3(2 * NT), lds, s, *a, n_tiles);
    }
    T3D_CHECK_LAUNCH();
    return T3D_OK;
  }
  if (a->N % 128 == 0 && (long)tiles_m * (a->N / 128) >= 512) {
// ... 24 lines not shown
      auto kern = k_pointmlp_bwd_r<DBN, TK, TN_, PR_>;                                             \
      allow_lds(reinterpret_cast<const void*>(kern), lds_with(lds, r));                            \
      T3D_LAUNCH(kern, grid, dim3(NT), lds_with(lds, r), s, *d, *w, n_w, *r);                      \
    } else {                                                                                       \
      auto kern = k_pointmlp_bwd<DBN, TK, TN_, PR_>;                                               \
      allow_lds(reinterpret_cast<const void*>(kern), lds);                                         \
      T3D_LAUNCH(kern, grid, dim3(NT), lds, s, *d, *w, n_w);                                       \
    }                                                                                              \
  } while (0)
#define T3D_BWDX(DBN, TK, TN_) do { if (d->w_x3 && d->N <= X3_CTAB_MAX_CH) T3D_BWDX_P(DBN, TK, TN_, PathX3P); else T3D_BWDX_P(DBN, TK, TN_, PathX3); } while (0)
#define T3D_BWDX_W(DBN)                                  \
  do {                                                   \
    if (tk == 128 && tn == 128) T3D_BWDX(DBN, 128, 128); \
    else if (tk == 128) T3D_BWDX(DBN, 128, 64);          \
    else if (tn == 128) T3D_BWDX(DBN, 64, 128);          \
    else T3D_BWDX(DBN, 64, 64);                          \
  } while (0)
  if (wide) T3D_BWDX_W(128);
  else T3D_BWDX_W(64);
#undef T3D_BWDX_W
#undef T3D_BWDX
#undef T3D_BWDX_P
  T3D_CHECK_LAUNCH();
  return T3D_OK;
}

int t3d_x3_stage1(const t3d_pointmlp_gram_args* g, const t3d_act_colsum_args* c, const t3d_pool_bwd_prep_args* q, const t3d_rider_set* r,
                  int gt, int n_gram, int n_colsum, int n_prep, size_t lds_other, hipStream_t s) {
  const dim3 grid(n_gram + n_colsum + n_prep + (r ? r->n_wg : 0));
  const size_t lds = lds_with(lds_max(lds_wgrad_x3(gt, gt), lds_other), r);
#define T3D_ST1X(GT_)                                                                  \
  do {                                                                                 \
    if (r) {                                                                           \
      auto kern = k_pool_bwd_stage1_r<GT_, PathX3>;                                    \
      allow_lds(reinterpret_cast<const void*>(kern), lds);                             \
      T3D_LAUNCH(kern, grid, dim3(NT), lds, s, *g, *c, *q, n_gram, n_colsum, *r);      \
    } else {                                                                           \
      auto kern = k_pool_bwd_stage1<GT_, PathX3>;                                      \
      allow_lds(reinterpret_cast<const void*>(kern), lds);                             \
      T3D_LAUNCH(kern, grid, dim3(NT), lds, s, *g, *c, *q, n_gram, n_colsum);          \
    }                                                                                  \
  } while (0)
  if (gt != 64) return T3D_ERR_ARG;
  T3D_ST1X(64);
#undef T3D_ST1X
  T3D_CHECK_LAUNCH();
  return T3D_OK;
}

int t3d_x3_stage2(const t3d_pool_wgrad_finish_args* f, const t3d_pointmlp_dgrad_gram_args* d, const t3d_rider_set* r, bool wide,
                  int n_finish, int n_d, size_t lds_other, hipStream_t s) {
  const dim3 grid(n_finish + n_d + (r ? r->n_wg : 0));
  const size_t lds = lds_with(lds_max(wide ? lds_fwd_x3(128) : lds_fwd_x3(64), lds_other), r);
#define T3D_ST2X(BN_)                                                                  \
  do {                                                                                 \
    if (r) {                                                                           \
      auto kern = k_pool_bwd_stage2_r<BN_, PathX3>;                                    \
      allow_lds(reinterpret_cast<const void*>(kern), lds);                             \
      T3D_LAUNCH(kern, grid, dim3(NT), lds, s, *f, *d, n_finish, *r);                  \
    } else {                                                                           \
      auto kern = k_pool_bwd_stage2<BN_, PathX3>;                                      \
      allow_lds(reinterpret_cast<const void*>(kern), lds);                             \
      T3D_LAUNCH(kern, grid, dim3(NT), lds, s, *f, *d, n_finish);                      \
    }                                                                                  \
  } while (0)
  if (wide) T3D_ST2X(128); else T3D_ST2X(64);
#undef T3D_ST2X
  T3D_CHECK_LAUNCH();
  return T3D_OK;
}
#else

#define T3D_QUERY_STREAM (reinterpret_cast<t3d_stream_t>(static_cast<intptr_t>(-1)))
#define T3D_HOSTED(r, stream) do { if ((stream) == T3D_QUERY_STREAM) return (r) ? 1 : 0; } while (0)
#define T3D_RIDERS_FIRST(r, stream)                         \
  do {                                                      \
    if ((stream) == T3D_QUERY_STREAM) return 0;             \
    if (r) {                                                \
      const int rc__ = t3d_run_riders(r, stream);           \
      if (rc__ != T3D_OK) return rc__;                      \
    }                                                       \
  } while (0)

extern "C" int t3d_pointmlp_fwd(const t3d_pointmlp_fwd_args* a, t3d_stream_t stream) { return t3d_pointmlp_fwd_r(a, nullptr, stream); }

extern "C" int t3d_pointmlp_fwd_r(const t3d_pointmlp_fwd_args* a, const t3d_rider_set* r, t3d_stream_t stream) {
  T3D_ABI_TAKE(pointmlp_fwd_args, a);
  if (a && a->struct_size != sizeof(*a)) return T3D_ERR_ABI;
  if (r && !riders_ok(r)) return T3D_ERR_ARG;
  if (!a || !a->w || !a->psum || !a->psumsq || !act_ok(a->a, a->K)) return T3D_ERR_ARG;
  if (a->pmax && (!a->pmin || !a->pamax || !a->pamin)) return T3D_ERR_ARG;
  if (a->M <= 0 || a->K <= 0 || a->N <= 0 || a->M % T3D_TILE_ROWS || a->rows_per_frustum % T3D_TILE_ROWS ||
      a->M % a->rows_per_frustum || a->N % 64 || (long)a->M * a->N >= (1L << 30))
    return T3D_ERR_SHAPE;
  hipStream_t s = static_cast<hipStream_t>(stream);
  const int tiles_m = a->M / 128;
  const bool sub = a->a.sub != nullptr;
  if (!dtype_ok(a->dtype)) return T3D_ERR_ARG;
  if (a->dtype == T3D_BF16) {
    T3D_RIDERS_FIRST(r, stream);
    const bool wide = a->N % 128 == 0 && (long)tiles_m * (a->N / 128) >= 512;
    const bool xh = a->a.dtype == T3D_BF16;
    if (xh && a->K % BKH) return T3D_ERR_SHAPE;
    static const bool use_tiny = []() { const char* e = getenv("T3D_FWD_TINYK"); return !(e && e[0] == '0'); }();
    if (use_tiny && !xh && a->K <= 4 && a->y && !a->pmax && !a->rowbias && (a->N == 64 || a->N == 128) && a->a.ldx % 4 == 0 &&
        a->a.coff % 4 == 0 && a->a.coff + 4 <= a->a.ldx) {
      if (a->N == 64) T3D_LAUNCH(k_pointmlp_fwd_tinyk<64>, dim3(tiles_m), dim3(NT), 0, s, *a);
      else T3D_LAUNCH(k_pointmlp_fwd_tinyk<128>, dim3(tiles_m), dim3(NT), 0, s, *a);
      T3D_CHECK_LAUNCH();
      return T3D_OK;
    }
    static const bool use_res = []() { const char* e = getenv("T3D_FWD_RES"); return !(e && e[0] == '0'); }();
    if (use_res && xh && !sub && (a->K == 64 || a->K == 128)) {
      static const int res_wgs = []() { const char* e = getenv("T3D_FWD_RES_WGS"); return e ? atoi(e) : 512; }();
      const dim3 grid(res_wgs > 0 && tiles_m > res_wgs ? res_wgs : tiles_m);
#define T3D_FWD_RES(BN_, KT_)                                                                                    \
  do {                                                                                                          \
    constexpr size_t lds = ((size_t)KT_ * 128 * LDRH + 2 * (size_t)BKH * (BN_ + 32)) * 2;                        \
    launch_lds(k_pointmlp_fwd_res<BN_, KT_>, grid, lds, s, *a);                                                 \
  } while (0)
      if (a->N % 128 == 0) { if (a->K == 64) T3D_FWD_RES(128, 1); else T3D_FWD_RES(128, 2); }
      else { if (a->K == 64) T3D_FWD_RES(64, 1); else T3D_FWD_RES(64, 2); }
#undef T3D_FWD_RES
      T3D_CHECK_LAUNCH();
      return T3D_OK;
    }
    const dim3 grid(tiles_m * (a->N / (wide ? 128 : 64)));
    const size_t lds = wide ? lds_fwd_h(128) : lds_fwd_h(64);
#define T3D_FWD_H(BN_)                                                                                          \
  do {                                                                                                          \
    if (sub) launch_lds(k_pointmlp_fwd<BN_, true, PathBF16, float>, grid, lds, s, *a);                          \
    else if (xh) launch_lds(k_pointmlp_fwd<BN_, false, PathBF16, bf16_t>, grid, lds, s, *a);                    \
    else launch_lds(k_pointmlp_fwd<BN_, false, PathBF16, float>, grid, lds, s, *a);                             \
  } while (0)
    if (wide) T3D_FWD_H(128);
    else T3D_FWD_H(64);
#undef T3D_FWD_H
    T3D_CHECK_LAUNCH();
    return T3D_OK;
  }
  if (a->a.dtype != T3D_F32) return T3D_ERR_ARG;
  {
    static const bool use_tiny32 = []() { const char* e = getenv("T3D_FWD_TINYK"); return !(e && e[0] == '0'); }();
    if (use_tiny32 && a->K <= 4 && a->y && !a->pmax && !a->rowbias && (a->N == 64 || a->N == 128) && a->a.ldx % 4 == 0 &&
        a->a.coff % 4 == 0 && a->a.coff + 4 <= a->a.ldx) {
      T3D_RIDERS_FIRST(r, stream);
      if (a->N == 64) T3D_LAUNCH((k_pointmlp_fwd_tinyk<64, float>), dim3(tiles_m), dim3(NT), 0, s, *a);
      else T3D_LAUNCH((k_pointmlp_fwd_tinyk<128, float>), dim3(tiles_m), dim3(NT), 0, s, *a);
      T3D_CHECK_LAUNCH();
      return T3D_OK;
    }
  }
  if (!sub && a->K % BKX == 0 && x3_layer(a->arith, a->K, a->N)) {
    T3D_HOSTED(r, stream);
    return t3d_x3_fwd(a, r, s);
  }
  static const bool use_pool_kernel = []() { const char* e = getenv("T3D_FWD_POOL"); return !(e && e[0] == '0'); }();
  static const bool fp_k256 = []() { const char* e = getenv("T3D_FWD_POOL"); return e && e[0] == '2'; }();
  if (use_pool_kernel && !a->y && a->pmax && !sub && a->N % 128 == 0 && a->N >= 256 && (a->K == 128 || (a->K == 256 && fp_k256))) {
    T3D_RIDERS_FIRST(r, stream);
#ifndef T3D_FP_WAVES
#define T3D_FP_WAVES 8
#endif
    if (a->K == 128) {
      auto kern = k_pointmlp_fwd_pool<128, 32, T3D_FP_WAVES>;
      constexpr size_t lds = FwdPool<128, 32, T3D_FP_WAVES>::LDS_BYTES;
      allow_lds(reinterpret_cast<const void*>(kern), lds);
      T3D_LAUNCH(kern, dim3(tiles_m), dim3(64 * T3D_FP_WAVES), lds, s, *a);
    } else {
      auto kern = k_pointmlp_fwd_pool<256, 16, T3D_FP_WAVES>;
      constexpr size_t lds = FwdPool<256, 16, T3D_FP_WAVES>::LDS_BYTES;
      allow_lds(reinterpret_cast<const void*>(kern), lds);
      T3D_LAUNCH(kern, dim3(tiles_m), dim3(64 * T3D_FP_WAVES), lds, s, *a);
    }
    T3D_CHECK_LAUNCH();
    return T3D_OK;
  }
  T3D_HOSTED(r, stream);
  if (a->N % 128 == 0 && (long)tiles_m * (a->N / 128) >= 512) {
    const dim3 grid(tiles_m * (a->N / 128) + (r ? r->n_wg : 0));
    if (r) {
      if (sub) launch_lds_r(k_pointmlp_fwd_r<128, true>, grid, lds_with(lds_fwd(128), r), s, *a, *r);
      else launch_lds_r(k_pointmlp_fwd_r<128, false>, grid, lds_with(lds_fwd(128), r), s, *a, *r);
    } else if (sub) launch_lds(k_pointmlp_fwd<128, true>, grid, lds_fwd(128), s, *a);
    else launch_lds(k_pointmlp_fwd<128, false>, grid, lds_fwd(128), s, *a);
  } else {
    const dim3 grid(tiles_m * (a->N / 64) + (r ? r->n_wg : 0));
    if (r) {
      if (sub) launch_lds_r(k_pointmlp_fwd_r<64, true>, grid, lds_with(lds_fwd(64), r), s, *a, *r);
      else launch_lds_r(k_pointmlp_fwd_r<64, false>, grid, lds_with(lds_fwd(64), r), s, *a, *r);
    } else if (sub) launch_lds(k_pointmlp_fwd<64, true>, grid, lds_fwd(64), s, *a);
    else launch_lds(k_pointmlp_fwd<64, false>, grid, lds_fwd(64), s, *a);
  }
  T3D_CHECK_LAUNCH();
  return T3D_OK;
}

static int check_dgrad(const t3d_pointmlp_dgrad_args* a) {
  if (a && a->struct_size != sizeof(*a)) return T3D_ERR_ABI;
  if (!a || !a->w || !a->out || !dy_ok(a->dy)) return T3D_ERR_ARG;
  if (a->prev_y && (!a->prev_scale || !a->prev_shift)) return T3D_ERR_ARG;
  if (a->psum_dz && (!a->psum_dzy || !a->prev_y)) return T3D_ERR_ARG;
  if (!dtype_ok(a->dtype) || a->dtype != a->dy.dtype) return T3D_ERR_ARG;
  if (a->M <= 0 || a->M % T3D_TILE_ROWS || a->rows_per_frustum % T3D_TILE_ROWS || a->M % a->rows_per_frustum ||
      a->K % 64 || a->N % 4 || (long)a->M * a->K >= (1L << 30) || (a->dtype == T3D_BF16 && a->N % 64))
    return T3D_ERR_SHAPE;
  return T3D_OK;
}
static bool dgrad_wide(const t3d_pointmlp_dgrad_args* a) {
  return a->K % 128 == 0 && (long)(a->M / 128) * (a->K / 128) >= 512;
}

extern "C" int t3d_pointmlp_dgrad(const t3d_pointmlp_dgrad_args* a, t3d_stream_t stream) {
  T3D_ABI_TAKE(pointmlp_dgrad_args, a);
  const int rc = check_dgrad(a);
  if (rc != T3D_OK) return rc;
  hipStream_t s = static_cast<hipStream_t>(stream);
  const int tiles_m = a->M / 128;
  const bool pooled = a->dy.dz == nullptr;
  if (a->dtype == T3D_BF16) {
    if (dgrad_wide(a)) launch_lds(k_pointmlp_dgrad<128, false, PathBF16>, dim3(tiles_m * (a->K / 128)), lds_dgrad_h(128), s, *a);
    else launch_lds(k_pointmlp_dgrad<64, false, PathBF16>, dim3(tiles_m * (a->K / 64)), lds_dgrad_h(64), s, *a);
    T3D_CHECK_LAUNCH();
    return T3D_OK;
  }
  if (!pooled && a->N % BKX == 0 && x3_layer_bwd(a->arith, a->K, a->N)) return t3d_x3_dgrad(a, dgrad_wide(a), s);
  if (dgrad_wide(a)) {
    const dim3 grid(tiles_m * (a->K / 128));
// ... 441 lines not shown
  T3D_CHECK_LAUNCH();
  return T3D_OK;
}

extern "C" int t3d_pool_bwd_stage2(const t3d_pool_wgrad_finish_args* f, const t3d_pointmlp_dgrad_gram_args* d,
                                   t3d_stream_t stream) {
  return t3d_pool_bwd_stage2_r(f, d, nullptr, stream);
}

extern "C" int t3d_pool_bwd_stage2_r(const t3d_pool_wgrad_finish_args* f, const t3d_pointmlp_dgrad_gram_args* d,
                                     const t3d_rider_set* r, t3d_stream_t stream) {
  T3D_ABI_TAKE(pointmlp_dgrad_gram_args, d);
  if (r && !riders_ok(r)) return T3D_ERR_ARG;
  int rc = check_finish(f);
  if (rc != T3D_OK) return rc;
  if ((rc = check_dgrad_gram(d)) != T3D_OK) return rc;
  hipStream_t s = static_cast<hipStream_t>(stream);
  const int n_finish = (f->K / FK) * (f->N / FN);
  if (f->a.dtype != d->a.dtype) return T3D_ERR_ARG;
  if (dgram1_ok(d) && f->K == d->K) {
    T3D_RIDERS_FIRST(r, stream);
    const int n_fin2 = (n_finish + 1) / 2, tiles = d->M / 128;
    const dim3 grid2(n_fin2 + (tiles < 256 ? tiles : 256));
    const int fin_floats = (int)(finish_lds(f->K) / sizeof(float));
#define T3D_ST2H(K_, BM_)                                                                                  \
  do {                                                                                                     \
    const size_t lds2 = lds_max(lds_dgram1(K_, BM_), 2 * finish_lds(K_));                                  \
    auto kern = k_pool_bwd_stage2_h<K_, BM_>;                                                              \
    allow_lds(reinterpret_cast<const void*>(kern), lds2);                                                  \
    T3D_LAUNCH(kern, grid2, dim3(NT1), lds2, s, *f, *d, n_fin2, fin_floats);                               \
  } while (0)
    if (d->K == 128) T3D_ST2H(128, 128); else T3D_ST2H(256, 64);
#undef T3D_ST2H
    T3D_CHECK_LAUNCH();
    return T3D_OK;
  }
  const bool wide = dgrad_gram_wide(d);
  const int n_d = (d->M / 128) * (d->K / (wide ? 128 : 64));
  const bool bf16 = d->dtype == T3D_BF16;
  if (f->a.dtype != d->a.dtype) return T3D_ERR_ARG;
  if (bf16) { T3D_RIDERS_FIRST(r, stream); r = nullptr; }
  const dim3 grid(n_finish + n_d + (r ? r->n_wg : 0));
  size_t lds = bf16 ? (wide ? lds_dgram_h(128) : lds_dgram_h(64)) : (wide ? lds_fwd(128) : lds_fwd(64));
  if (finish_lds(f->K) > lds) lds = finish_lds(f->K);
  T3D_HOSTED(r, stream);
  if (!bf16 && d->K % BKX == 0 && x3_layer_bwd(d->arith, d->K, d->K)) return t3d_x3_stage2(f, d, r, wide, n_finish, n_d, finish_lds(f->K), s);
  lds = lds_with(lds, r);
#define T3D_ST2(BN_, PR_)                                                              \
  do {                                                                                 \
    auto kern = k_pool_bwd_stage2<BN_, PR_>;                                           \
    allow_lds(reinterpret_cast<const void*>(kern), lds);                               \
    T3D_LAUNCH(kern, grid, dim3(NT), lds, s, *f, *d, n_finish);                        \
  } while (0)
#define T3D_ST2R(BN_)                                                                  \
  do {                                                                                 \
    auto kern = k_pool_bwd_stage2_r<BN_>;                                              \
    allow_lds(reinterpret_cast<const void*>(kern), lds);                               \
    T3D_LAUNCH(kern, grid, dim3(NT), lds, s, *f, *d, n_finish, *r);                    \
  } while (0)
  if (r) { if (wide) T3D_ST2R(128); else T3D_ST2R(64); }
  else if (bf16) { if (wide) T3D_ST2(128, PathBF16); else T3D_ST2(64, PathBF16); }
  else { if (wide) T3D_ST2(128, PathF32); else T3D_ST2(64, PathF32); }
#undef T3D_ST2R
#undef T3D_ST2
  T3D_CHECK_LAUNCH();
  return T3D_OK;
}

extern "C" int t3d_split_x3(const float* src, void* planes, int64_t n, int64_t plane_stride, t3d_stream_t stream) {
  if (!src || !planes || n <= 0 || plane_stride < n || (reinterpret_cast<uintptr_t>(src) & 15) || (reinterpret_cast<uintptr_t>(planes) & 7) ||
      (plane_stride & 3))
    return T3D_ERR_ARG;
  return t3d_x3_split(src, planes, n, plane_stride, static_cast<hipStream_t>(stream));
}

extern "C" int t3d_split_x3_frag(const float* params, void* planes_fwd, void* planes_dgrad, int64_t plane_stride, const t3d_x3_frag_entry* table,
                                 int n_entries, int n_blocks, t3d_stream_t stream) {
  if (!params || !planes_fwd || !planes_dgrad || !table || n_entries <= 0 || n_blocks <= 0 || plane_stride <= 0 || (plane_stride & 7) ||
      (reinterpret_cast<uintptr_t>(params) & 15) || (reinterpret_cast<uintptr_t>(planes_fwd) & 15) || (reinterpret_cast<uintptr_t>(planes_dgrad) & 15))
    return T3D_ERR_ARG;
  return t3d_x3_split_frag(params, planes_fwd, planes_dgrad, plane_stride, table, n_entries, n_blocks, static_cast<hipStream_t>(stream));
}

static const t3d_rider_set* query_set() {
  static const t3d_rider_set q = []() { t3d_rider_set r{}; r.n_ops = 1; r.n_wg = 1; r.sync = reinterpret_cast<unsigned*>(16); return r; }();
  return &q;
}
extern "C" int t3d_gemm_arithmetic(int arith, int dtype, int K, int N, int kind) {
  if (dtype == T3D_BF16) return T3D_ARITH_BF16;
  bool x3 = false;
  switch (kind) {
    case T3D_GEMM_FWD: x3 = K % BKX == 0 && x3_layer(arith, K, N); break;
    case T3D_GEMM_BWD: x3 = N % BKX == 0 && K % 64 == 0 && (K <= 64 || K % 128 == 0) && x3_layer_bwd(arith, K, N); break;
    case T3D_GEMM_DGRAD: x3 = N % BKX == 0 && x3_layer_bwd(arith, K, N); break;
    case T3D_GEMM_WGRAD: x3 = K % 64 == 0 && (K <= 64 || K % 128 == 0) && x3_layer_bwd(arith, K, N); break;
    case T3D_GEMM_GRAM: x3 = x3_layer_bwd(arith, K, K); break;
    case T3D_GEMM_DGRAD_GRAM: x3 = K % BKX == 0 && x3_layer_bwd(arith, K, K); break;
    default: return T3D_ERR_ARG;
  }
  return x3 ? T3D_ARITH_BF16X3 : T3D_ARITH_FP32_MFMA;
}
extern "C" int t3d_pointmlp_fwd_hosts_riders(const t3d_pointmlp_fwd_args* a) { return t3d_pointmlp_fwd_r(a, query_set(), T3D_QUERY_STREAM); }
extern "C" int t3d_pointmlp_wgrad_hosts_riders(const t3d_pointmlp_wgrad_args* a) { return t3d_pointmlp_wgrad_r(a, query_set(), T3D_QUERY_STREAM); }
extern "C" int t3d_pointmlp_bwd_hosts_riders(const t3d_pointmlp_dgrad_args* d, const t3d_pointmlp_wgrad_args* w) {
  return t3d_pointmlp_bwd_r(d, w, query_set(), T3D_QUERY_STREAM);
}
extern "C" int t3d_pool_bwd_stage1_hosts_riders(const t3d_pointmlp_gram_args* g, const t3d_act_colsum_args* c, const t3d_pool_bwd_prep_args* q) {
  return t3d_pool_bwd_stage1_r(g, c, q, query_set(), T3D_QUERY_STREAM);
}
extern "C" int t3d_pool_bwd_stage2_hosts_riders(const t3d_pool_wgrad_finish_args* f, const t3d_pointmlp_dgrad_gram_args* d) {
  return t3d_pool_bwd_stage2_r(f, d, query_set(), T3D_QUERY_STREAM);
}

#ifdef T3D_TRACE
int t3d_x3_set_trace(void* buf);
extern "C" int t3d_set_trace(void* buf) {
  unsigned long long* p = static_cast<unsigned long long*>(buf);
  if (t3d_x3_set_trace(buf) != T3D_OK) return T3D_ERR_LAUNCH;
  return hipMemcpyToSymbol(HIP_SYMBOL(t3d_trace_ptr), &p, sizeof(p)) == hipSuccess ? T3D_OK : T3D_ERR_LAUNCH;
}
#endif

#endif
#if defined(T3D_X3_TU) && defined(T3D_TRACE)
int t3d_x3_set_trace(void* buf) {
  unsigned long long* p = static_cast<unsigned long long*>(buf);
  return hipMemcpyToSymbol(HIP_SYMBOL(t3d_trace_ptr), &p, sizeof(p)) == hipSuccess ? T3D_OK : T3D_ERR_LAUNCH;
}
#endif
```

### transferable3d_amd/engine.py

```python
import contextlib
import ctypes as C
import math
import os

import numpy as np
import torch

from . import abi
from .abi import fptr, iptr
from .constants import BN_EPS

TILE = abi.TILE_ROWS


class Runtime:

    def __init__(self, device=None, lib=None, gemm_arithmetic=None):
        self.lib = lib if lib is not None else abi.load()
        if gemm_arithmetic is None:
            gemm_arithmetic = 'fp32_mfma' if os.environ.get('T3D_X3', '1') == '0' else 'bf16x3'
        self.gemm_arithmetic = gemm_arithmetic
        self.arith = abi.ARITH_BY_NAME[gemm_arithmetic]
        if device is None:
            if not torch.cuda.is_available():
                raise abi.T3DError('no GPU visible: the product path runs on an MI355X only')
            device = torch.device('cuda', torch.cuda.current_device())
        self.device = torch.device(device)
        self.allocs = []
        self._side = None

    def side_stream(self):
        if self._side is None:
            self._side = torch.cuda.Stream(self.device)
        return self._side

    def stream(self):
        if self.device.type == 'cuda':
            return C.c_void_p(torch.cuda.current_stream(self.device).cuda_stream)
        return C.c_void_p(0)

    def zeros(self, *shape, dtype=torch.float32):
        t = torch.zeros(*shape, dtype=dtype, device=self.device)
        self.allocs.append(t)
        return t

    def full(self, shape, val, dtype=torch.float32):
        t = torch.full(shape, val, dtype=dtype, device=self.device)
        self.allocs.append(t)
        return t


SIDE_STREAM = os.environ.get('T3D_SIDE_STREAM', '0') == '1'
FUSE_BWD = os.environ.get('T3D_FUSE_BWD', '1') != '0'
FC_SIDE = os.environ.get('T3D_FC_SIDE', '0') == '1'
SPARSE_GATED = os.environ.get('T3D_SPARSE_GATED', '1') != '0'
DZ_POOL = os.environ.get('T3D_DZ_POOL', '0') == '1' and not SIDE_STREAM and not FC_SIDE and FUSE_BWD


class Plan:

    JOIN, FLUSH = '__join__', '__flush__'
    MARK = '__mark__'
    BUCKET, WAIT = '__bucket__', '__wait__'

    def __init__(self, rt):
        self.rt = rt
        self.calls = []
        self.lanes = []
        self.keep = []
        self._lane = 0
        self.two_streams = False

    @contextlib.contextmanager
    def side(self):
        prev, self._lane = self._lane, 1
        try:
            yield self
        finally:
            self._lane = prev

    def add(self, name, args):
        fn = getattr(self.rt.lib, name)
        ref = C.byref(args)
        self.keep.append(args)
        self.calls.append((name, lambda s, fn=fn, ref=ref: fn(ref, s), args))
        self.lanes.append(self._lane)

    def add_raw(self, name, thunk, *keep):
        self.keep.extend(keep)
        self.calls.append((name, thunk, None))
        self.lanes.append(self._lane)

    def mark(self, tag):
        self.calls.append((Plan.MARK, lambda s: 0, tag))
        self.lanes.append(0)

    def join(self):
        self.calls.append((Plan.JOIN, lambda s: 0, None))
        self.lanes.append(0)

    def flush(self):
        self.calls.append((Plan.FLUSH, lambda s: 0, None))
        self.lanes.append(0)

    def run(self):
        if self.rt.device.type == 'cuda' and any(self.lanes) and (SIDE_STREAM or self.two_streams):
            return self._run_two_streams()
        s = self.rt.stream()
        for name, call, _ in self.calls:
            rc = call(s)
            if rc != 0:
                abi.check(rc, name)

    def _run_two_streams(self):
        main, side = torch.cuda.current_stream(self.rt.device), self.rt.side_stream()
        ms, ss = C.c_void_p(main.cuda_stream), C.c_void_p(side.cuda_stream)
        deferred, pending = [], False

        def issue_side():
            nonlocal pending
            if deferred:
                side.wait_stream(main)
                for name, call in deferred:
                    rc = call(ss)
                    if rc != 0:
                        abi.check(rc, name)
                del deferred[:]
                pending = True

        for (name, call, _), lane in zip(self.calls, self.lanes):
            if name == Plan.FLUSH:
                issue_side()
            elif name == Plan.JOIN:
                issue_side()
                if pending:
                    main.wait_stream(side)
                pending = False
            elif lane == 1:
                deferred.append((name, call))
            else:
                rc = call(ms)
                if rc != 0:
                    abi.check(rc, name)
        issue_side()
        if pending:
            main.wait_stream(side)

    def bucket_ready(self, i):
        self.calls.append((Plan.BUCKET, lambda s: 0, i))
        self.lanes.append(0)

    def bucket_wait(self, i):
        self.calls.append((Plan.WAIT, lambda s: 0, i))
        self.lanes.append(0)

    def __len__(self):
        return sum(1 for name, _, _ in self.calls if not name.startswith('__'))


X3_PRESPLIT = os.environ.get('T3D_X3', '1') != '0' and os.environ.get('T3D_X3_PRESPLIT', '1') == '1'


class VarStore:

    def __init__(self, rt, capacity=4 << 20, state_capacity=1 << 16, seed=0):
        self.rt = rt
        self.params = rt.zeros(capacity)
        self.grads = rt.zeros(capacity)
        self.adam_m = rt.zeros(capacity)
        self.adam_v = rt.zeros(capacity)
        self.state = rt.zeros(state_capacity)
        self.params16 = None
        self.used = 0
# ... 663 lines not shown
```

### transferable3d_amd/nets.py

```python
import ctypes as C
import os

import numpy as np
import torch

from . import abi
from .abi import fptr, iptr
from .constants import BOX_OUT_DIMS, NUM_CLASS
from .engine import ActSpec, FcLayer, Plan, PointLayer, Runtime, VarStore, Workspace, TILE


class Graph:

    def __init__(self, batch_size, num_point, num_channel, rt=None, seed=0, unbiased_ema=True, vars=None, dtype='f32'):
        assert dtype in ('f32', 'bf16')
        self.dtype = dtype
        self.dt = abi.DTYPE_BY_NAME[dtype]
        self.adt = torch.bfloat16 if dtype == 'bf16' else torch.float32
        if num_point % TILE:
            raise abi.T3DError('num_point must be a multiple of %d' % TILE)
        self.rt = rt or Runtime()
        self.B, self.rpf, self.C = batch_size, num_point, num_channel
        self.ldpc = (num_channel + 3) // 4 * 4
        self.M = batch_size * num_point
        self.vars = vars or VarStore(self.rt, seed=seed)
        self.ws = Workspace(self.rt)
        self.unbiased_ema = unbiased_ema
        self.hyper = self.rt.zeros(4)
        self.hyper[2] = 0.5
        self.bn_decay_ptr = self.hyper[2:3]
        self.dropout_masks = {}
        self.inline_dropout, self.dropout_seed = False, 1234
        self.deferred_slab_ptrs = []
        self.dp_buckets = False
        self.buckets = []
        self.trained_prefixes = None
        self._slabs_reduced = 0
        self.fwd = Plan(self.rt)
        self.bwd = Plan(self.rt)
        self.opt = Plan(self.rt)
        self.pre = Plan(self.rt)
        self.finalized = False

    def finalize(self):
        self.ws.finalize()
        base = self.ws.buf.data_ptr()
        for a, field, soff in self.deferred_slab_ptrs:
            setattr(a, field, C.cast(C.c_void_p(base + 4 * soff), abi.F))
        self.finalized = True
        return self

    def emit_reduce_slabs(self, plan):
        ws, vs, lib = self.ws, self.vars, self.rt.lib
        plan.join()
        i0, i1 = self._slabs_reduced, len(ws.entries)
        self._slabs_reduced = i1
        if i1 == i0:
            return
        mx = max(e[2] for e in ws.entries[i0:i1])
        stride = C.sizeof(abi.SlabDesc)

        def thunk(s):
            return lib.t3d_reduce_slabs(fptr(ws.buf), fptr(vs.grads),
                                        C.cast(C.c_void_p(ws.table.data_ptr() + i0 * stride), C.POINTER(abi.SlabDesc)), i1 - i0, mx, s)
        plan.add_raw('t3d_reduce_slabs', thunk)

    def emit_cast_weights(self, plan):
        vs, lib = self.vars, self.rt.lib
        if self.dt != abi.BF16:
            from .engine import X3_PRESPLIT
            if (X3_PRESPLIT and self.rt.device.type == 'cuda' and self.rt.arith != abi.ARITH_FP32_MFMA and getattr(vs, 'x3_frag_enabled', True)
                    and hasattr(lib, 't3d_split_x3_frag')):
                def thunk(s):
                    if not getattr(vs, 'x3_frag_entries', None):
                        return 0
                    t, n, nblk = vs.frag_table()
                    pf, pd = vs.x3_frag_planes
                    return lib.t3d_split_x3_frag(fptr(vs.params), C.c_void_p(pf.data_ptr()), C.c_void_p(pd.data_ptr()), vs.x3_frag_stride,
                                                 C.c_void_p(t.data_ptr()), n, nblk, s)
                plan.add_raw('t3d_split_x3_frag', thunk)
            return
        p16 = vs.enable_bf16()
        plan.add_raw('t3d_cast_bf16', lambda s: lib.t3d_cast_bf16(fptr(vs.params), C.c_void_p(p16.data_ptr()), vs.used, s))

    def default_bucket(self):
        return self.vars.trainable_ranges(self.trained_prefixes)

    def declare_bucket(self, plan, prefixes):
        if not self.dp_buckets:
            return
        self.emit_reduce_slabs(plan)
        self.buckets.append(self.vars.trainable_ranges(prefixes))
        plan.bucket_ready(len(self.buckets) - 1)

    def emit_batch_assemble(self, plan, dataset, inputs, seed=0, **aug):
        equal_prob = aug.pop('equal_class_prob', 0.0)
        semi = aug.pop('semi_sampling', None)
        if semi is not None:
            slots = self.rt.zeros(self.B, dtype=torch.int32)
            plan.add('t3d_semi_sample', dataset.semi_sample_args(self.hyper, self.B, slots, inputs.is_data_2D, method=semi,
                                                                 seed=seed ^ 0x2545F491, equal_prob=equal_prob))
            if aug.pop('alternate', False):
                raise ValueError('alternate=True (the two-list walk of split_by_class) and semi_sampling=%r exclude each other' % semi)
            a = dataset.assemble_args(inputs, self.hyper, self.B, self.rpf, self.C, seed=seed, sample=slots, **aug)
            a.is_data_2D, a.frustum_is_2D, a.slot_is_2D = iptr(None), iptr(None), iptr(inputs.is_data_2D)
            plan.add('t3d_batch_assemble', a)
            return
        if equal_prob > 0.0:
            slots = self.rt.zeros(self.B, dtype=torch.int32)
            alternate = bool(aug.pop('alternate', False))
            plan.add('t3d_sample_equal_classes', dataset.sample_equal_args(
                self.hyper, self.B, slots, is_data_2D=inputs.is_data_2D if alternate else None, seed=seed ^ 0x2545F491,
                equal_prob=equal_prob, alternate=alternate))
            a = dataset.assemble_args(inputs, self.hyper, self.B, self.rpf, self.C, seed=seed, sample=slots, **aug)
            if alternate:
                a.is_data_2D = iptr(None)
                a.slot_is_2D = iptr(inputs.is_data_2D)
            plan.add('t3d_batch_assemble', a)
            return
        a = dataset.assemble_args(inputs, self.hyper, self.B, self.rpf, self.C, seed=seed, **aug)
        plan.add('t3d_batch_assemble', a)

    def emit_boxpc_perturb(self, plan, inputs, c, seed=0):
        from .dataset import boxpc_perturb_args
        plan.add('t3d_boxpc_perturb', boxpc_perturb_args(inputs, self.hyper, self.B, c, seed=seed))

    def emit_schedule(self, plan, sched):
        lib, hyper = self.rt.lib, self.hyper
        plan.add_raw('t3d_schedule_step', lambda s: lib.t3d_schedule_step(fptr(hyper), C.byref(sched), s), sched)

    def emit_dropout_masks(self, plan, seed=1234):
        lib, hyper = self.rt.lib, self.hyper
        for i, (scope, (mask, keep)) in enumerate(sorted(self.dropout_masks.items())):
            plan.add_raw('t3d_dropout_mask',
                         lambda s, mask=mask, keep=keep, sd=seed + 7919 * i: lib.t3d_dropout_mask(
                             fptr(mask), mask.numel(), keep, sd, fptr(hyper), s))

    def emit_adam(self, plan, prefixes=None, beta1=0.9, beta2=0.999, eps=1e-8, grad_scale=1.0):
        lib, vs, hyper = self.rt.lib, self.vars, self.hyper
        vs.optimizer_kind = 'adam'

        def adam(off, n):
            plan.add_raw('t3d_adam_tf_step',
                         lambda s, off=off, n=n: lib.t3d_adam_tf_step(
                             fptr(vs.params[off:]), fptr(vs.grads[off:]), fptr(vs.adam_m[off:]), fptr(vs.adam_v[off:]),
                             n, fptr(hyper), beta1, beta2, eps, grad_scale, s))
        self._emit_optimizer(plan, prefixes, adam)

    def emit_momentum(self, plan, prefixes=None, momentum=0.9, grad_scale=1.0):
        lib, vs, hyper = self.rt.lib, self.vars, self.hyper
        vs.optimizer_kind = 'momentum'

        def mom(off, n):
            plan.add_raw('t3d_momentum_step',
                         lambda s, off=off, n=n: lib.t3d_momentum_step(
                             fptr(vs.params[off:]), fptr(vs.grads[off:]), fptr(vs.adam_m[off:]), n, fptr(hyper), momentum, grad_scale, s))
        self._emit_optimizer(plan, prefixes, mom)

    def _emit_optimizer(self, plan, prefixes, launch):
        vs = self.vars
        self.trained_prefixes = prefixes
        ranges = vs.trainable_ranges(prefixes)
        if self.buckets:
            covered = sorted(r for b in self.buckets for r in b)
            assert sum(n for _, n in covered) == sum(n for _, n in ranges) and \
                all(any(o >= ro and o + n <= ro + rn for ro, rn in ranges) for o, n in covered), \
                'gradient buckets must partition the trained variables'
            for i, b in enumerate(self.buckets):
                plan.bucket_wait(i)
                for off, n in b:
                    launch(off, n)
            return
        for off, n in ranges:
            launch(off, n)


def make_schedule(batch_size, base_lr=1e-3, decay_step=800000, decay_rate=0.5, bn_init_decay=0.5,
                  bn_decay_rate=0.5, bn_decay_clip=0.99, beta1=0.9, beta2=0.999):
    return abi.Schedule(base_lr, decay_rate, float(decay_step), bn_init_decay, bn_decay_rate, float(decay_step),
                        bn_decay_clip, beta1, beta2, batch_size, 0)


class InstSegNet:
    def __init__(self, g, scope, use_one_hot):
        self.g, self.scope = g, scope
        C_, vs = g.C, g.vars
        s = scope + '/'
        self.L1 = PointLayer(g, s + 'conv1', C_, 64, kernel_1xD=True)
        self.L2 = PointLayer(g, s + 'conv2', 64, 64)
        self.L3 = PointLayer(g, s + 'conv3', 64, 64)
        self.L4 = PointLayer(g, s + 'conv4', 64, 128)
        self.L5 = PointLayer(g, s + 'conv5', 128, 1024, pool=True)
        self.oh = NUM_CLASS if use_one_hot else 0
        k6 = 64 + 1024 + self.oh
        w6 = vs.xavier(s + 'conv6/weights', (1, 1, k6, 512), k6, 512).view(k6, 512)
        self.L6 = PointLayer(g, s + 'conv6', 64, 512, w=w6[0:64], w_name=s + 'conv6/weights', w_row0=0)
        self.G6 = FcLayer(g, s + 'conv6/global', 1024, 512, bn=False, act=None, K2=self.oh, w=w6[64:], bias=None)
        self.G6.w_grad = vs.grad(s + 'conv6/weights').view(k6, 512)[64:]
        self.L7 = PointLayer(g, s + 'conv7', 512, 256)
        self.L8 = PointLayer(g, s + 'conv8', 256, 128)
        self.L9 = PointLayer(g, s + 'conv9', 128, 128)
        self.w10 = vs.xavier(s + 'conv10/weights', (1, 1, 128, 2), 128, 2).view(128, 2)
        self.b10 = vs.const(s + 'conv10/biases', (2,), 0.0)
        rt, M, T, B = g.rt, g.M, g.M // TILE, g.B
        self.drop_mask = None
        if not g.inline_dropout:
            self.drop_mask = rt.full((M, 128), 1.0)
            g.dropout_masks[s + 'dp1'] = (self.drop_mask, 0.5)
        self.logits, self.mask = rt.zeros(M, 2), rt.zeros(M)
        self.part = rt.zeros(T, 8)
        self.mask_xyz_mean, self.seg_loss, self.n_correct = rt.zeros(B, 3), rt.zeros(B), rt.zeros(1)

    def fwd(self, plan, pc, one_hot, labels, is_data_2D, is_training, train_seg, ce_weight=1.0, oracle_mask=None):
        g, rt = self.g, self.g.rt
        M, T = g.M, g.M // TILE
        a = ActSpec(pc, g.ldpc, g.C)
        a = self.L1.fwd(plan, a, is_training)
        a = self.L2.fwd(plan, a, is_training)
        a3 = self.L3.fwd(plan, a, is_training)
        a = self.L4.fwd(plan, a3, is_training)
        self.L5.fwd(plan, a, is_training)
        rb = self.G6.fwd(plan, self.L5.pooled, 1024, is_training, in2=one_hot if self.oh else None, ld_in2=NUM_CLASS)
        a = self.L6.fwd(plan, a3, is_training, rowbias=rb)
        a = self.L7.fwd(plan, a, is_training)
        a = self.L8.fwd(plan, a, is_training)
        self.L9.fwd(plan, a, is_training)
        self.train_seg = train_seg
        h = abi.SegHeadArgs()
        L9 = self.L9
# ... 913 lines not shown
```

### transferable3d_amd/step.py

```python
import os

import torch

from . import abi
from .engine import Plan


OPTIMIZER_CALLS = ('t3d_adam_tf_step', 't3d_momentum_step')


class TrainStep:
    def __init__(self, engine, pre, fwd, bwd=None, opt=None, process_group=None, use_hip_graph=None, force_dist=False,
                 one_graph=None):
        self.e, self.rt = engine, engine.rt
        self.pre, self.fwd, self.bwd, self.opt = pre, fwd, bwd, opt
        self.train = bwd is not None
        self.pg = process_group
        self.world = process_group.size() if process_group is not None else 1
        self.dist = self.train and process_group is not None and (self.world > 1 or force_dist)
        self.on_gpu = self.rt.device.type == 'cuda'
        want = use_hip_graph if use_hip_graph is not None else self.on_gpu
        self.want_graph = bool(want) and self.on_gpu
        env = os.environ.get('T3D_DP_ONE_GRAPH', '')
        if one_graph is None:
            if env in ('0', '1', '2'):
                one_graph = env != '0'
            else:
                one_graph = self.dist and self.on_gpu and self._backend() == 'nccl' and self.world == 1
        self.one_graph = bool(one_graph) and self.dist and self.on_gpu
        self.one_graph_form = env if env in ('1', '2') else None
        self.cache = {}
        self.n_runs = 0
        self._capture_stream = None
        self.time_waits = False
        self._wait_events = []
        self._sets = None
        self.schedule_report = None
        self.rider_check_every = int(os.environ.get('T3D_RIDER_CHECK_EVERY', '64'))

    def _backend(self):
        try:
            import torch.distributed as dist
            return str(dist.get_backend(self.pg)).lower()
        except Exception:
            return ''

    def _buckets(self):
        b = list(getattr(self.e, 'buckets', []))
        return b if b else [self.e.default_bucket()]

    def _program(self, generate_masks):
        plans = ([self.pre] if self.pre is not None else []) + [self.fwd] + ([self.bwd, self.opt] if self.train else [])
        calls, lanes, two = [], [], False
        for p in plans:
            for (name, call, arg), lane in zip(p.calls, p.lanes):
                if name == 't3d_dropout_mask' and not generate_masks:
                    continue
                calls.append((name, call, arg))
                lanes.append(lane)
            calls.append((Plan.JOIN, lambda s: 0, None))
            lanes.append(0)
            two = two or p.two_streams
        if self.dist and not any(c[0] == Plan.BUCKET for c in calls):
            k = next((i for i, c in enumerate(calls) if c[0] in OPTIMIZER_CALLS), len(calls))
            calls[k:k] = [(Plan.BUCKET, lambda s: 0, 0), (Plan.WAIT, lambda s: 0, 0)]
            lanes[k:k] = [0, 0]
        if not two:
            calls, lanes = self._overlap(calls, lanes)
            two = two or getattr(self, 'two_stream', False)
        prog, cur = [], Plan(self.rt)
        cur.two_streams = two

        def close():
            nonlocal cur
            if len(cur):
                prog.append(('run', cur))
            cur = Plan(self.rt)
            cur.two_streams = two

        for (name, call, arg), lane in zip(calls, lanes):
            if name in (Plan.BUCKET, Plan.WAIT):
                if self.dist:
                    close()
                    prog.append(('allreduce' if name == Plan.BUCKET else 'wait', arg))
                continue
            cur.calls.append((name, call, arg))
            cur.lanes.append(lane)
        close()
        k = len(prog)
        while k > 0 and (prog[k - 1][0] == 'wait' or (prog[k - 1][0] == 'run' and
                                                      all(c[0] in OPTIMIZER_CALLS + (Plan.JOIN,) for c in prog[k - 1][1].calls))):
            k -= 1
        tail = prog[k:]
        if sum(1 for kind, _ in tail if kind == 'run') > 1:
            merged = Plan(self.rt)
            merged.two_streams = two
            for kind, x in tail:
                if kind == 'run':
                    merged.calls.extend(x.calls)
                    merged.lanes.extend(x.lanes)
            prog = prog[:k] + [t for t in tail if t[0] == 'wait'] + [('run', merged)]
        return prog

    def _overlap(self, calls, lanes):
        from . import schedule
        tags = {c[2]: i for i, c in enumerate(calls) if c[0] == Plan.MARK}
        if not all(t in tags for t in ('T_begin', 'S_begin', 'S_end')) or not hasattr(self.rt.lib, 't3d_pointmlp_bwd_r'):
            return calls, lanes
        tb, sb, se = tags['T_begin'], tags['S_begin'], tags['S_end']
        if not tb < sb < se:
            return calls, lanes
        if self._shares_gpu():
            return calls, lanes
        real = lambda cs: [c for c in cs if not c[0].startswith('__')]
        if any(c[0] in (Plan.BUCKET, Plan.WAIT) for c in calls[tb:se]):
            return calls, lanes
        S_calls, T_calls = real(calls[sb:se]), real(calls[tb:sb])
        if self._two_stream_overlap(S_calls + T_calls):
            self.two_stream = True
            first, second = (T_calls, S_calls) if os.environ.get('T3D_TWO_STREAM_FIRST', 'S') == 'T' else (S_calls, T_calls)
            lanes2 = [0] * tb + [1] * len(first) + [0] + [0] * len(second) + [0]
            merged = first + [(Plan.FLUSH, lambda s: 0, None)] + second + [(Plan.JOIN, lambda s: 0, None)]
            calls = calls[:tb] + merged + calls[se + 1:]
            lanes2 += [0] * (len(calls) - len(lanes2))
            self.schedule_report = {'mode': 'two streams', 'S_launches': len(S_calls), 'T_launches': len(T_calls), 'hosted': 0, 'rider_ops': 0,
                                    'pairs': 0, 'solo': len(S_calls) + len(T_calls)}
            return calls, lanes2
        if self._sets is None:
            self._sets = schedule.RiderSets(self.rt)
        merged, self.schedule_report = schedule.overlap_chains(self.rt, S_calls, T_calls, self._sets)
        return calls[:tb] + merged + calls[se + 1:], lanes[:tb] + [0] * len(merged) + lanes[se + 1:]

    def _two_stream_overlap(self, chain_calls):
        mode = os.environ.get('T3D_OVERLAP_STREAMS', '')
        if mode in ('0', '1'):
            return mode == '1' and self.on_gpu
        if not self.on_gpu:
            return False
        return self.e.M >= 4 * 32768

    def _shares_gpu(self):
        if not self.on_gpu or os.environ.get('T3D_RIDERS_SHARED_GPU', '0') == '1':
            return False
        local_ranks = int(os.environ.get('LOCAL_WORLD_SIZE', self.world))
        return local_ranks > torch.cuda.device_count()

    def rider_timeouts(self):
        return self._sets.timeouts() if self._sets is not None else 0

    def check_riders(self):
        if self._sets is not None:
            self._sets.check()

    def _allreduce(self, i, async_op):
        import torch.distributed as dist
        g = self.e.vars.grads
        works = []
        for off, n in self._buckets()[i]:
            works.append(dist.all_reduce(g[off:off + n], group=self.pg, async_op=async_op))
        return works

    def _run_program(self, prog, graphs=None):
        pending = {}
        for k, (kind, x) in enumerate(prog):
            if kind == 'run':
                if graphs is not None and graphs.get(k) is not None:
                    graphs[k].replay()
                else:
                    x.run()
            elif kind == 'allreduce':
                pending[x] = self._allreduce(x, async_op=self.on_gpu)
            else:
                ev = None
                if self.time_waits and self.on_gpu:
                    ev = (torch.cuda.Event(enable_timing=True), torch.cuda.Event(enable_timing=True))
                    ev[0].record()
                for w in pending.pop(x, []):
                    if w is not None:
                        w.wait()
                if ev is not None:
                    ev[1].record()
                    self._wait_events.append(ev)
        for ws in pending.values():
            for w in ws:
                if w is not None:
# ... 43 lines not shown
                if seen and first_only:
                    continue
                seen = True
                g = torch.cuda.CUDAGraph()
                with torch.cuda.graph(g, stream=s, capture_error_mode='thread_local'):
                    x.run()
                graphs[k] = g
        return prog, graphs

    def run(self, generate_masks=True):
        self.n_runs += 1
        self._issue(generate_masks)
        if self._sets is not None and self.rider_check_every > 0 and self.n_runs % self.rider_check_every == 0:
            self.check_riders()

    def _issue(self, generate_masks):
        key = bool(generate_masks)
        ent = self.cache.get(key)
        if ent is None:
            ent = self.cache[key] = {'prog': self._program(key), 'graphs': None, 'runs': 0}
        ent['runs'] += 1
        if not self.want_graph or ent['runs'] == 1:
            return self._run_program(ent['prog'])
        if ent['graphs'] is None:
            prog, graphs = self._capture(ent['prog'])
            ent['cprog'], ent['graphs'] = prog, graphs
            if self._sets is not None:
                self._sets.timeouts()
        if ent['cprog'] and ent['cprog'][0][0] == 'run_graph':
            ent['graphs'][0].replay()
            return
        self._run_program(ent['cprog'], ent['graphs'])

    def dp_report(self):
        mode = 'flat' if len(self._buckets()) == 1 else 'bucketed'
        if self.one_graph:
            mode += ', the step and its collectives captured in ONE graph'
        else:
            mode += ', host-issued collectives between graph segments'
        exposed = None
        if self._wait_events:
            torch.cuda.synchronize()
            n_wait = max(1, sum(1 for kind, _ in self.cache[True]['prog'] if kind == 'wait'))
            steps = max(1, len(self._wait_events) // n_wait)
            exposed = sum(a.elapsed_time(b) for a, b in self._wait_events) * 1e3 / steps
        if getattr(self, 'one_graph_fallback', None):
            mode += ' (one-graph capture failed: %s)' % self.one_graph_fallback
        return {'mode': mode, 'world': self.world, 'gradient_buckets': len(self._buckets()),
                'bucket_floats': [sum(n for _, n in b) for b in self._buckets()],
                'exposed_allreduce_us_per_step': exposed}

    def n_launches(self):
        return sum(len(p) for p in ([self.pre] if self.pre is not None else []) + [self.fwd] + ([self.bwd, self.opt] if self.train else []))

    def n_graph_segments(self, generate_masks=True):
        ent = self.cache.get(bool(generate_masks))
        if ent is None or ent['graphs'] is None:
            return 0
        return len(ent['graphs'])


WORKLOADS = ('A', 'boxpc', 'F')


def workload_flags(workload):
    from .config import make_parser
    if workload == 'A':
        c = make_parser().parse_special_args(['--SEMI_MODEL', 'A', '--WEAK_WEIGHT_REPROJECTION', '0', '--WEAK_WEIGHT_SURFACE', '0'])
        import os
        c.WEAK_LOSS_SUMMARIES = os.environ.get('T3D_WEAK_SUMMARIES', '0') == '1'
        return c
    if workload == 'boxpc':
        return make_parser().parse_special_args(['--BOX_PC_MASK_REPRESENTATION', 'A', '--BOXPC_WEIGHT_DELTA', '4'])
    return make_parser().parse_special_args(
        ['--SEMI_MODEL', 'F', '--BOX_PC_MASK_REPRESENTATION', 'A', '--WEAK_WEIGHT_INTRACLASSVAR', '2', '--WEAK_WEIGHT_REPROJECTION', '0',
         '--SEMI_MULTIPLIER_FOR_WEAK_LOSS', '0.05', '--SEMI_BOXPC_FIT_ONLY_ON_2D_CLS', '1', '--SEMI_WEIGHT_BOXPC_FIT_LOSS', '1'])


STAGE_C_TRAIN_CLASSES = [i in (1, 2, 6, 7, 8) for i in range(10)]


def build_training_step(rt, workload, B, N, C, world=1, rank=0, process_group=None, force_dist=False, flat_allreduce=False,
                        use_hip_graph=None, inline_dropout=True, dropout_seed=1234, seed=0, state_dict=None, c=None, dtype='f32',
                        one_graph=None):
    from .nets import BoxPCModel, Graph, SemiModelA, SemiModelF, make_schedule
    assert workload in WORKLOADS
    g = Graph(B, N, C, rt=rt, seed=seed, dtype=dtype)
    g.inline_dropout, g.dropout_seed = inline_dropout, dropout_seed + rank
    c = c if c is not None else workload_flags(workload)
    prefixes = None
    if workload == 'A':
        model = SemiModelA(g, c)
        loss = model.loss_op.loss
    elif workload == 'boxpc':
        model = BoxPCModel(g, c, False)
        loss = model.loss_op.loss
    else:
        model = SemiModelF(g, c, use_one_hot=True, train_classes=STAGE_C_TRAIN_CLASSES)
        loss = model.loss
        prefixes = list(SemiModelF.VAR_LIST)
    if state_dict is not None:
        g.vars.load_state_dict(state_dict)
    dist_on = process_group is not None and (world > 1 or force_dist)
    g.dp_buckets = dist_on and not flat_allreduce
    g.emit_schedule(g.pre, make_schedule(B * world))
    g.emit_dropout_masks(g.pre, seed=dropout_seed + rank)
    if workload == 'F':
        model.emit_forward(g.fwd, True, True, train=True)
    else:
        model.emit_forward(g.fwd, True, True)
    model.emit_backward(g.bwd)
    g.emit_adam(g.opt, prefixes=prefixes, grad_scale=1.0 / world)
    g.finalize()
    step = TrainStep(g, g.pre, g.fwd, g.bwd, g.opt, process_group=process_group, use_hip_graph=use_hip_graph,
                     force_dist=force_dist, one_graph=one_graph)
    return g, model, step, loss


class _Program:

    def __init__(self, rt, calls, want_graph):
        self.plan = Plan(rt)
        self.plan.calls, self.plan.lanes = list(calls), [0] * len(calls)
        self.want_graph, self.runs, self.graph = want_graph, 0, None

    def run(self, stream_holder):
        self.runs += 1
        if not self.want_graph or self.runs == 1:
            return self.plan.run()
        if self.graph is None:
            torch.cuda.synchronize()
            if stream_holder[0] is None:
                stream_holder[0] = torch.cuda.Stream()
            g = torch.cuda.CUDAGraph()
            with torch.cuda.graph(g, stream=stream_holder[0], capture_error_mode='thread_local'):
                self.plan.run()
            self.graph = g
        self.graph.replay()


class PipelinedStep:

    def __init__(self, rt, ctxs, use_hip_graph=None):
        from . import schedule
        self.rt, self.ctxs = rt, ctxs
        self.on_gpu = rt.device.type == 'cuda'
        self.want_graph = (bool(use_hip_graph) if use_hip_graph is not None else self.on_gpu) and self.on_gpu
        self.dist, self.world, self.time_waits = False, 1, False
        self._sets = schedule.RiderSets(rt)
        self.rider_check_every = int(os.environ.get('T3D_RIDER_CHECK_EVERY', '64'))
        self._stream = [None]
        self.n_runs = 0
        self.fwd_pending = False
        ch = [self._chains(c) for c in ctxs]
        mk = lambda calls: _Program(rt, calls, self.want_graph)
        self.head, self.steady, self.tail, self.reports = [], [], [], []
        for i in (0, 1):
            me, nxt = ch[i], ch[1 - i]
            self.head.append(mk(me['pre'] + me['F']))
            t_chain = me['Tf'] + me['Tb'] + me['adam_T']
            calls, rep = schedule.overlap_chains(rt, me['S'] + me['reduce_S'] + me['adam_S'] + nxt['pre'] + nxt['F'], t_chain, self._sets)
            self.steady.append(mk(calls))
            self.reports.append(rep)
            calls, _ = schedule.overlap_chains(rt, me['S'] + me['reduce_S'] + me['adam_S'], t_chain, self._sets)
            self.tail.append(mk(calls))
        self.schedule_report = self.reports[0]

    @staticmethod
    def _chains(ctx):
        g = ctx['g']
        real = lambda cs: [c for c in cs if not c[0].startswith('__')]

        def split(calls, tag):
            k = next(i for i, c in enumerate(calls) if c[0] == Plan.MARK and c[2] == tag)
            return calls[:k], calls[k + 1:]
        F, Tf = split(g.fwd.calls, 'T_begin')
        Tb, rest = split(g.bwd.calls, 'S_begin')
        S, after = split(rest, 'S_end')
        return dict(pre=real(g.pre.calls), F=real(F), Tf=real(Tf), Tb=real(Tb), S=real(S), reduce_S=real(after),
                    adam_T=real(ctx['opt_T'].calls), adam_S=real(ctx['opt_S'].calls))

    def inputs(self, k=None):
        return self.ctxs[(self.n_runs if k is None else k) % 2]['model'].inputs

    def loss(self, k):
        return self.ctxs[k % 2]['loss']

    def run(self, last=False):
        i = self.n_runs % 2
        if not self.fwd_pending:
            self.head[i].run(self._stream)
        (self.tail if last else self.steady)[i].run(self._stream)
        self.fwd_pending = not last
        self.n_runs += 1
        if self.rider_check_every > 0 and self.n_runs % self.rider_check_every == 0:
            self.check_riders()

    def profile_plans(self):
# ... 49 lines not shown
```

Before: 27460.

## Fuse step head kernels and fold Adam into slab gradient reduction

Adds a fused head kernel that runs the LR/BN schedule update, the bf16x3 weight fragment split and the first tiny-K point-MLP forward in one launch. It also adds a fused tail kernel that reduces the gradient slabs and applies the Adam update in the same pass, with extra blocks covering parameter ranges that are not slab-reduced. The aim is to cut kernel launches and a full re-read of gradients in the optimizer. The cost is more complex kernels, and a dependency risk if the forward blocks read hyper or the split planes that the head kernel writes in the same launch. It is enabled by default through an env flag and only applies under certain conditions (bf16x3, non-distributed, f32).

```diff
diff --git a/include/t3d.h b/include/t3d.h
--- a/include/t3d.h
+++ b/include/t3d.h
@@ -728,6 +728,11 @@
                      const float* hyper, float beta1, float beta2, float eps, float grad_scale,
                      t3d_stream_t stream);
 
+typedef struct { int64_t off; int64_t n; int32_t blk0; int32_t reserved; } t3d_adam_range;
+int t3d_reduce_slabs_adam(const float* slab_base, float* grad_base, const t3d_slab_desc* table_dev, int n_tensors, int max_numel,
+                          float* params, float* m, float* v, const t3d_adam_range* ranges_dev, int n_ranges, int n_range_blocks,
+                          const float* hyper, float beta1, float beta2, float eps, float grad_scale, t3d_stream_t stream);
+
 int t3d_split_x3(const float* src, void* planes, int64_t n, int64_t plane_stride, t3d_stream_t stream);
 
 typedef struct {
@@ -739,6 +744,11 @@
 } t3d_x3_frag_entry;
 int t3d_split_x3_frag(const float* params, void* planes_fwd, void* planes_dgrad, int64_t plane_stride, const t3d_x3_frag_entry* table,
                       int n_entries, int n_blocks, t3d_stream_t stream);
+
+int t3d_step_head_takes(const t3d_pointmlp_fwd_args* fwd);
+int t3d_step_head(const t3d_pointmlp_fwd_args* fwd, const float* params, void* planes_fwd, void* planes_dgrad, int64_t plane_stride,
+                  const t3d_x3_frag_entry* table, int n_entries, int n_blocks, float* hyper, const t3d_schedule* sched,
+                  t3d_stream_t stream);
 
 int t3d_momentum_step(float* params, const float* grads, float* accum, int64_t n, const float* hyper, float momentum,
                       float grad_scale, t3d_stream_t stream);
diff --git a/transferable3d_amd/abi.py b/transferable3d_amd/abi.py
--- a/transferable3d_amd/abi.py
+++ b/transferable3d_amd/abi.py
@@ -235,6 +235,29 @@
 
 class SlabDesc(C.Structure):
     _fields_ = [('slab_off', C.c_int64), ('grad_off', C.c_int64), ('numel', C.c_int32), ('n_slabs', C.c_int32)]
+
+
+class AdamRange(C.Structure):
+    _fields_ = [('off', C.c_int64), ('n', C.c_int64), ('blk0', C.c_int32), ('reserved', C.c_int32)]
+
+
+ADAM_RANGE_ELEMS = 1024
+
+
+def adam_range_table(n_total, slab_tensors):
+    out, pos, blk = [], 0, 0
+    for off, n in sorted(slab_tensors):
+        if n <= 0 or off < pos or off + n > n_total:
+            raise T3DError('slab tensors overlap or leave the parameter buffer: (%d, %d) after %d of %d' % (off, n, pos, n_total))
+        if off > pos:
+            out.append((pos, off - pos, blk))
+            blk += (off - pos + ADAM_RANGE_ELEMS - 1) // ADAM_RANGE_ELEMS
+        pos = off + n
+    if pos < n_total:
+        out.append((pos, n_total - pos, blk))
+        blk += (n_total - pos + ADAM_RANGE_ELEMS - 1) // ADAM_RANGE_ELEMS
+    assert sum(n for _, n, _ in out) + sum(n for _, n in slab_tensors) == n_total
+    return out, blk
 
 
 class Schedule(C.Structure):
@@ -426,6 +449,9 @@
     't3d_anchor_reg_bwd': [C.POINTER(AnchorRegBwdArgs), VP],
     't3d_reduce_slabs': [F, F, C.POINTER(SlabDesc), i32, i32, VP],
     't3d_schedule_step': [F, C.POINTER(Schedule), VP],
+    't3d_reduce_slabs_adam': [F, F, C.POINTER(SlabDesc), i32, i32, F, F, F, C.POINTER(AdamRange), i32, i32, F, f32, f32, f32, f32, VP],
+    't3d_step_head_takes': [C.POINTER(PointMlpFwdArgs)],
+    't3d_step_head': [C.POINTER(PointMlpFwdArgs), F, VP, VP, C.c_int64, VP, i32, i32, F, C.POINTER(Schedule), VP],
     't3d_adam_tf_step': [F, F, F, F, C.c_int64, F, f32, f32, f32, f32, VP],
     't3d_momentum_step': [F, F, F, C.c_int64, F, f32, f32, VP],
     't3d_split_x3': [F, VP, C.c_int64, C.c_int64, VP],
diff --git a/transferable3d_amd/csrc/bn_dev.h b/transferable3d_amd/csrc/bn_dev.h
--- a/transferable3d_amd/csrc/bn_dev.h
+++ b/transferable3d_amd/csrc/bn_dev.h
@@ -204,16 +204,44 @@
   p.out[i] = (float)((double)p.alpha * v);
 }
 
+__device__ __forceinline__ float adam_tf_elem(const float g, float& m, float& v, const float lr_t, const float b1, const float b2,
+                                              const float eps, const float gscale) {
+#pragma clang fp contract(off)
+  const float gi = g * gscale;
+  const float mi = b1 * m + (1.f - b1) * gi;
+  const float vi = b2 * v + (1.f - b2) * gi * gi;
+  m = mi;
+  v = vi;
+  return lr_t * mi / (sqrtf(vi) + eps);
+}
+
+struct adam_tail {
+  float* w;
+  float* m;
+  float* v;
+  const float* hyper;
+  float b1, b2, eps, gscale;
+};
+
+template <bool ADAM = false>
 __device__ __forceinline__ void reduce_slabs_body(const float* __restrict__ slab_base, float* __restrict__ grad_base,
                                                   const t3d_slab_desc* __restrict__ table, float4 (*part)[32], int bx, int by,
-                                                  int gx) {
+                                                  int gx, const adam_tail* ad = nullptr) {
   const t3d_slab_desc d = table[by];
+  float lr_t = 0.f;
+  if constexpr (ADAM) lr_t = ad->hyper[3];
   const bool vec = ((d.slab_off | d.grad_off | (int64_t)d.numel) & 3) == 0;
   const int n4 = vec ? (d.numel >> 2) : 0;
   const int el = threadIdx.x & 31, grp = threadIdx.x >> 5;
   for (int e0 = bx * 32; e0 < n4; e0 += gx * 32) {
     const int e = e0 + el;
     float4 a0 = make_float4(0.f, 0.f, 0.f, 0.f), a1 = a0, a2 = a0, a3 = a0;
+    float4 w4, m4, v4;
+    if constexpr (ADAM) if (grp == 0 && e < n4) {
+      w4 = reinterpret_cast<const float4*>(ad->w + d.grad_off)[e];
+      m4 = reinterpret_cast<const float4*>(ad->m + d.grad_off)[e];
+      v4 = reinterpret_cast<const float4*>(ad->v + d.grad_off)[e];
+    }
     if (e < n4) {
       const float4* s = reinterpret_cast<const float4*>(slab_base + d.slab_off) + e;
       int k = grp;
@@ -255,6 +283,15 @@
         t.x += u.x; t.y += u.y; t.z += u.z; t.w += u.w;
       }
       reinterpret_cast<float4*>(grad_base + d.grad_off)[e] = t;
+      if constexpr (ADAM) {
+        w4.x -= adam_tf_elem(t.x, m4.x, v4.x, lr_t, ad->b1, ad->b2, ad->eps, ad->gscale);
+        w4.y -= adam_tf_elem(t.y, m4.y, v4.y, lr_t, ad->b1, ad->b2, ad->eps, ad->gscale);
+        w4.z -= adam_tf_elem(t.z, m4.z, v4.z, lr_t, ad->b1, ad->b2, ad->eps, ad->gscale);
+        w4.w -= adam_tf_elem(t.w, m4.w, v4.w, lr_t, ad->b1, ad->b2, ad->eps, ad->gscale);
+        reinterpret_cast<float4*>(ad->m + d.grad_off)[e] = m4;
+        reinterpret_cast<float4*>(ad->v + d.grad_off)[e] = v4;
+        reinterpret_cast<float4*>(ad->w + d.grad_off)[e] = w4;
+      }
     }
     __syncthreads();
   }
@@ -263,9 +300,36 @@
       float acc = 0.f;
       for (int k = 0; k < d.n_slabs; ++k) acc += slab_base[d.slab_off + (size_t)k * d.numel + e];
       grad_base[d.grad_off + e] = acc;
-    }
-  }
-}
-
-
-}
+      if constexpr (ADAM) {
+        const size_t o = (size_t)d.grad_off + e;
+        float mi = ad->m[o], vi = ad->v[o];
+        const float dw = adam_tf_elem(acc, mi, vi, lr_t, ad->b1, ad->b2, ad->eps, ad->gscale);
+        ad->m[o] = mi;
+        ad->v[o] = vi;
+        ad->w[o] -= dw;
+      }
+    }
+  }
+}
+
+__device__ __forceinline__ void schedule_step_body(float* hyper, const t3d_schedule s, const int lane) {
+  const double step = (double)hyper[0] + (double)s.step_offset;
+  const double seen = step * (double)s.batch_size;
+  const double t = step + 1.0;
+  const double base = lane == 0 ? (double)s.lr_decay_rate : lane == 1 ? (double)s.bn_decay_rate : lane == 2 ? (double)s.beta2 : (double)s.beta1;
+  const double expo = lane == 0 ? floor(seen / (double)s.lr_decay_step) : lane == 1 ? floor(seen / (double)s.bn_decay_step) : t;
+  const double pw = lane < 4 ? pow(base, expo) : 0.0;
+  const double p_lr = __shfl(pw, 0), p_bn = __shfl(pw, 1), p_b2 = __shfl(pw, 2), p_b1 = __shfl(pw, 3);
+  if (lane != 0) return;
+  const double lr = (double)s.base_lr * p_lr;
+  const double bnm = (double)s.bn_init_decay * p_bn;
+  const double bnd = fmin((double)s.bn_decay_clip, 1.0 - bnm);
+  const double lr_t = lr * sqrt(1.0 - p_b2) / (1.0 - p_b1);
+  hyper[1] = (float)lr;
+  hyper[2] = (float)bnd;
+  hyper[3] = (float)lr_t;
+  hyper[0] = (float)t;
+}
+
+
+}
diff --git a/transferable3d_amd/csrc/bn_optim.hip b/transferable3d_amd/csrc/bn_optim.hip
--- a/transferable3d_amd/csrc/bn_optim.hip
+++ b/transferable3d_amd/csrc/bn_optim.hip
@@ -48,23 +48,7 @@
 
 __global__ __launch_bounds__(64) void k_schedule_step(float* hyper, const t3d_schedule s) {
   if (blockIdx.x != 0) return;
-  const int lane = threadIdx.x;
-  const double step = (double)hyper[0] + (double)s.step_offset;
-  const double seen = step * (double)s.batch_size;
-  const double t = step + 1.0;
-  const double base = lane == 0 ? (double)s.lr_decay_rate : lane == 1 ? (double)s.bn_decay_rate : lane == 2 ? (double)s.beta2 : (double)s.beta1;
-  const double expo = lane == 0 ? floor(seen / (double)s.lr_decay_step) : lane == 1 ? floor(seen / (double)s.bn_decay_step) : t;
-  const double pw = lane < 4 ? pow(base, expo) : 0.0;
-  const double p_lr = __shfl(pw, 0), p_bn = __shfl(pw, 1), p_b2 = __shfl(pw, 2), p_b1 = __shfl(pw, 3);
-  if (lane != 0) return;
-  const double lr = (double)s.base_lr * p_lr;
-  const double bnm = (double)s.bn_init_decay * p_bn;
-  const double bnd = fmin((double)s.bn_decay_clip, 1.0 - bnm);
-  const double lr_t = lr * sqrt(1.0 - p_b2) / (1.0 - p_b1);
-  hyper[1] = (float)lr;
-  hyper[2] = (float)bnd;
-  hyper[3] = (float)lr_t;
-  hyper[0] = (float)t;
+  schedule_step_body(hyper, s, threadIdx.x);
 }
 
 __global__ __launch_bounds__(256) void k_adam_tf(float* __restrict__ w, const float* __restrict__ g, float* __restrict__ m,
@@ -72,12 +56,45 @@
                                                  float b1, float b2, float eps, float gscale) {
   const float lr_t = hyper[3];
   for (int64_t i = (int64_t)blockIdx.x * blockDim.x + threadIdx.x; i < n; i += (int64_t)gridDim.x * blockDim.x) {
-    const float gi = g[i] * gscale;
-    const float mi = b1 * m[i] + (1.f - b1) * gi;
-    const float vi = b2 * v[i] + (1.f - b2) * gi * gi;
+    float mi = m[i], vi = v[i];
+    const float dw = adam_tf_elem(g[i], mi, vi, lr_t, b1, b2, eps, gscale);
     m[i] = mi;
     v[i] = vi;
-    w[i] -= lr_t * mi / (sqrtf(vi) + eps);
+    w[i] -= dw;
+  }
+}
+
+constexpr int ADAM_RANGE_ELEMS = 1024;
+__global__ __launch_bounds__(256) void k_reduce_slabs_adam(const float* __restrict__ slab_base, float* __restrict__ grad_base,
+                                                           const t3d_slab_desc* __restrict__ table, const int gx, const int n_reduce,
+                                                           const t3d_adam_range* __restrict__ ranges, const int n_ranges,
+                                                           const adam_tail ad) {
+  __shared__ float4 part[8][32];
+  const int b = blockIdx.x;
+  if (b < n_reduce) {
+    reduce_slabs_body<true>(slab_base, grad_base, table, part, b % gx, b / gx, gx, &ad);
+    return;
+  }
+  const int r = b - n_reduce;
+  int lo = 0, hi = n_ranges - 1;
+  while (lo < hi) {
+    const int mid = (lo + hi + 1) >> 1;
+    if (ranges[mid].blk0 <= r) lo = mid; else hi = mid - 1;
+  }
+  const t3d_adam_range rg = ranges[lo];
+  const float lr_t = ad.hyper[3];
+  const int64_t i0 = (int64_t)(r - rg.blk0) * ADAM_RANGE_ELEMS + threadIdx.x;
+#pragma unroll
+  for (int u = 0; u < ADAM_RANGE_ELEMS / 256; ++u) {
+    const int64_t i = i0 + 256 * u;
+    if (i < rg.n) {
+      const int64_t o = rg.off + i;
+      float mi = ad.m[o], vi = ad.v[o];
+      const float dw = adam_tf_elem(grad_base[o], mi, vi, lr_t, ad.b1, ad.b2, ad.eps, ad.gscale);
+      ad.m[o] = mi;
+      ad.v[o] = vi;
+      ad.w[o] -= dw;
+    }
   }
 }
 
@@ -197,6 +214,23 @@
   if (blocks > 2048) blocks = 2048;
   T3D_LAUNCH(k_adam_tf, dim3((unsigned)blocks), dim3(256), 0, static_cast<hipStream_t>(stream), params, grads, m,
                      v, n, hyper, beta1, beta2, eps, grad_scale);
+  T3D_CHECK_LAUNCH();
+  return T3D_OK;
+}
+
+extern "C" int t3d_reduce_slabs_adam(const float* slab_base, float* grad_base, const t3d_slab_desc* table_dev, int n_tensors,
+                                     int max_numel, float* params, float* m, float* v, const t3d_adam_range* ranges_dev, int n_ranges,
+                                     int n_range_blocks, const float* hyper, float beta1, float beta2, float eps, float grad_scale,
+                                     t3d_stream_t stream) {
+  if (!slab_base || !grad_base || !table_dev || n_tensors <= 0 || !params || !m || !v || !hyper) return T3D_ERR_ARG;
+  if (n_ranges < 0 || n_range_blocks < 0 || (n_ranges == 0) != (n_range_blocks == 0) || (n_ranges > 0 && !ranges_dev)) return T3D_ERR_ARG;
+  int gx = (max_numel / 4 + 31) / 32;
+  if (gx > 256) gx = 256;
+  if (gx < 1) gx = 1;
+  const int n_reduce = gx * n_tensors;
+  const adam_tail ad = {params, m, v, hyper, beta1, beta2, eps, grad_scale};
+  T3D_LAUNCH(k_reduce_slabs_adam, dim3(n_reduce + n_range_blocks), dim3(256), 0, static_cast<hipStream_t>(stream), slab_base, grad_base,
+             table_dev, gx, n_reduce, ranges_dev, n_ranges, ad);
   T3D_CHECK_LAUNCH();
   return T3D_OK;
 }
diff --git a/transferable3d_amd/csrc/pointmlp.hip b/transferable3d_amd/csrc/pointmlp.hip
--- a/transferable3d_amd/csrc/pointmlp.hip
+++ b/transferable3d_amd/csrc/pointmlp.hip
@@ -1781,13 +1781,12 @@
   T3D_TRACE_MARK8(7);
 }
 
-template <int N, class YT = bf16_t>
-__global__ __launch_bounds__(NT) void k_pointmlp_fwd_tinyk(const t3d_pointmlp_fwd_args p) {
+template <int N, class YT>
+__device__ __forceinline__ void pointmlp_fwd_tinyk_body(const t3d_pointmlp_fwd_args& p, float (*red)[NT / (N / 8)][N], const int tile) {
   constexpr bool H = Elem<YT>::BF16;
   constexpr int CPR = N / 8, RPP = NT / CPR, NP = 128 / RPP;
-  __shared__ float red[2][RPP][N];
   const int tid = threadIdx.x, ch = tid % CPR, r0 = tid / CPR;
-  const int tile = blockIdx.x, row0 = tile * 128, b = row0 / p.rows_per_frustum;
+  const int row0 = tile * 128, b = row0 / p.rows_per_frustum;
   float w[4][8], add[8];
 #pragma unroll
   for (int k = 0; k < 4; ++k) {
@@ -1863,6 +1862,12 @@
     p.psum[(size_t)tile * p.N + tid] = t1;
     p.psumsq[(size_t)tile * p.N + tid] = t2;
   }
+}
+
+template <int N, class YT = bf16_t>
+__global__ __launch_bounds__(NT) void k_pointmlp_fwd_tinyk(const t3d_pointmlp_fwd_args p) {
+  __shared__ float red[2][NT / (N / 8)][N];
+  pointmlp_fwd_tinyk_body<N, YT>(p, red, blockIdx.x);
 }
 
 struct DgradEpilogue {
@@ -3489,6 +3494,8 @@
                   int n_finish, int n_d, size_t lds_other, hipStream_t s);
 int t3d_x3_split(const float* src, void* planes, int64_t n, int64_t plane_stride, hipStream_t s);
 int t3d_x3_split_frag(const float* params, void* pf, void* pd, int64_t stride, const t3d_x3_frag_entry* tab, int n, int n_blocks, hipStream_t s);
+int t3d_x3_step_head(const t3d_pointmlp_fwd_args* a, const float* params, void* pf, void* pd, int64_t stride, const t3d_x3_frag_entry* tab, int n,
+                     int n_blocks, float* hyper, const t3d_schedule* sched, hipStream_t s);
 int t3d_x3_dgrad(const t3d_pointmlp_dgrad_args* a, bool wide, hipStream_t s);
 int t3d_x3_wgrad(const t3d_pointmlp_wgrad_args* a, int tk, int tn, int n_blocks, hipStream_t s);
 int t3d_x3_gram(const t3d_pointmlp_gram_args* a, int tk, int n_blocks, hipStream_t s);
@@ -3516,14 +3523,14 @@
 }
 }
 namespace {
-__global__ __launch_bounds__(256) void k_split_x3_frag(const float* __restrict__ params, bf16_t* __restrict__ pf, bf16_t* __restrict__ pd, long stride,
-                                                       const t3d_x3_frag_entry* __restrict__ tab, int n) {
+__device__ __forceinline__ void split_x3_frag_body(const float* __restrict__ params, bf16_t* __restrict__ pf, bf16_t* __restrict__ pd, long stride,
+                                                   const t3d_x3_frag_entry* __restrict__ tab, int n, const int blk) {
   int e = 0;
-  while (e + 1 < n && (int)blockIdx.x >= tab[e + 1].blk0) ++e;
+  while (e + 1 < n && blk >= tab[e + 1].blk0) ++e;
   const t3d_x3_frag_entry en = tab[e];
   const float* w = params + en.off;
   const long nfr = (long)en.K * en.N / 8;
-  const long f = (long)((int)blockIdx.x - en.blk0) * 256 + threadIdx.x;
+  const long f = (long)(blk - en.blk0) * 256 + threadIdx.x;
   if (f >= nfr) return;
   const int lane = (int)(f & 63);
   const long q = f >> 6;
@@ -3560,6 +3567,32 @@
     *reinterpret_cast<bf16x8*>(d + 2 * stride) = __builtin_shufflevector(l0, l1, 0, 1, 2, 3, 4, 5, 6, 7);
   }
 }
+__global__ __launch_bounds__(256) void k_split_x3_frag(const float* __restrict__ params, bf16_t* __restrict__ pf, bf16_t* __restrict__ pd, long stride,
+                                                       const t3d_x3_frag_entry* __restrict__ tab, int n) {
+  split_x3_frag_body(params, pf, pd, stride, tab, n, (int)blockIdx.x);
+}
+
+template <int N>
+__global__ __launch_bounds__(NT) void k_step_head(const t3d_pointmlp_fwd_args p, const int n_fwd, const float* __restrict__ params,
+                                                  bf16_t* __restrict__ pf, bf16_t* __restrict__ pd, const long stride,
+                                                  const t3d_x3_frag_entry* __restrict__ tab, const int n, const int n_split, float* hyper,
+                                                  const t3d_schedule sched) {
+  __shared__ float red[2][NT / (N / 8)][N];
+  const int b = blockIdx.x;
+  if (b < n_fwd) pointmlp_fwd_tinyk_body<N, float>(p, red, b);
+  else if (b < n_fwd + n_split) split_x3_frag_body(params, pf, pd, stride, tab, n, b - n_fwd);
+  else if (threadIdx.x < 64) schedule_step_body(hyper, sched, threadIdx.x);
+}
+}
+int t3d_x3_step_head(const t3d_pointmlp_fwd_args* a, const float* params, void* pf, void* pd, int64_t stride, const t3d_x3_frag_entry* tab, int n,
+                     int n_blocks, float* hyper, const t3d_schedule* sched, hipStream_t s) {
+  static_assert(NT == 256, "the three roles of k_step_head are 256-thread workgroups");
+  const int n_fwd = a->M / 128;
+  const dim3 grid(n_fwd + n_blocks + 1);
+  if (a->N == 64) T3D_LAUNCH(k_step_head<64>, grid, dim3(NT), 0, s, *a, n_fwd, params, static_cast<bf16_t*>(pf), static_cast<bf16_t*>(pd), (long)stride, tab, n, n_blocks, hyper, *sched);
+  else T3D_LAUNCH(k_step_head<128>, grid, dim3(NT), 0, s, *a, n_fwd, params, static_cast<bf16_t*>(pf), static_cast<bf16_t*>(pd), (long)stride, tab, n, n_blocks, hyper, *sched);
+  T3D_CHECK_LAUNCH();
+  return T3D_OK;
 }
 int t3d_x3_split_frag(const float* params, void* pf, void* pd, int64_t stride, const t3d_x3_frag_entry* tab, int n, int n_blocks, hipStream_t s) {
   T3D_LAUNCH(k_split_x3_frag, dim3(n_blocks), dim3(256), 0, s, params, static_cast<bf16_t*>(pf), static_cast<bf16_t*>(pd), (long)stride, tab, n);
@@ -3750,6 +3783,12 @@
     }                                                       \
   } while (0)
 
+static bool fwd_takes_tinyk32(const t3d_pointmlp_fwd_args* a) {
+  static const bool use_tiny32 = []() { const char* e = getenv("T3D_FWD_TINYK"); return !(e && e[0] == '0'); }();
+  return use_tiny32 && a->K <= 4 && a->y && !a->pmax && !a->rowbias && (a->N == 64 || a->N == 128) && a->a.ldx % 4 == 0 &&
+         a->a.coff % 4 == 0 && a->a.coff + 4 <= a->a.ldx;
+}
+
 extern "C" int t3d_pointmlp_fwd(const t3d_pointmlp_fwd_args* a, t3d_stream_t stream) { return t3d_pointmlp_fwd_r(a, nullptr, stream); }
 
 extern "C" int t3d_pointmlp_fwd_r(const t3d_pointmlp_fwd_args* a, const t3d_rider_set* r, t3d_stream_t stream) {
@@ -3809,9 +3848,7 @@
   }
   if (a->a.dtype != T3D_F32) return T3D_ERR_ARG;
   {
-    static const bool use_tiny32 = []() { const char* e = getenv("T3D_FWD_TINYK"); return !(e && e[0] == '0'); }();
-    if (use_tiny32 && a->K <= 4 && a->y && !a->pmax && !a->rowbias && (a->N == 64 || a->N == 128) && a->a.ldx % 4 == 0 &&
-        a->a.coff % 4 == 0 && a->a.coff + 4 <= a->a.ldx) {
+    if (fwd_takes_tinyk32(a)) {
       T3D_RIDERS_FIRST(r, stream);
       if (a->N == 64) T3D_LAUNCH((k_pointmlp_fwd_tinyk<64, float>), dim3(tiles_m), dim3(NT), 0, s, *a);
       else T3D_LAUNCH((k_pointmlp_fwd_tinyk<128, float>), dim3(tiles_m), dim3(NT), 0, s, *a);
@@ -4419,6 +4456,33 @@
   return t3d_x3_split_frag(params, planes_fwd, planes_dgrad, plane_stride, table, n_entries, n_blocks, static_cast<hipStream_t>(stream));
 }
 
+static int step_head_fwd_check(const t3d_pointmlp_fwd_args* a) {
+  if (!a || !a->w || !a->psum || !a->psumsq || !act_ok(a->a, a->K)) return T3D_ERR_ARG;
+  if (a->M <= 0 || a->K <= 0 || a->N <= 0 || a->M % T3D_TILE_ROWS || a->rows_per_frustum % T3D_TILE_ROWS ||
+      a->M % a->rows_per_frustum || a->N % 64 || (long)a->M * a->N >= (1L << 30))
+    return T3D_ERR_SHAPE;
+  if (a->dtype != T3D_F32 || a->a.dtype != T3D_F32 || !fwd_takes_tinyk32(a) || a->a.scale || a->a.shift || a->a.sub) return T3D_ERR_ARG;
+  return T3D_OK;
+}
+
+extern "C" int t3d_step_head_takes(const t3d_pointmlp_fwd_args* a) {
+  T3D_ABI_TAKE(pointmlp_fwd_args, a);
+  return step_head_fwd_check(a) == T3D_OK ? 1 : 0;
+}
+
+extern "C" int t3d_step_head(const t3d_pointmlp_fwd_args* a, const float* params, void* planes_fwd, void* planes_dgrad, int64_t plane_stride,
+                             const t3d_x3_frag_entry* table, int n_entries, int n_blocks, float* hyper, const t3d_schedule* sched,
+                             t3d_stream_t stream) {
+  T3D_ABI_TAKE(pointmlp_fwd_args, a);
+  if (!hyper || !sched) return T3D_ERR_ARG;
+  if (!params || !planes_fwd || !planes_dgrad || !table || n_entries <= 0 || n_blocks <= 0 || plane_stride <= 0 || (plane_stride & 7) ||
+      (reinterpret_cast<uintptr_t>(params) & 15) || (reinterpret_cast<uintptr_t>(planes_fwd) & 15) || (reinterpret_cast<uintptr_t>(planes_dgrad) & 15))
+    return T3D_ERR_ARG;
+  const int rc = step_head_fwd_check(a);
+  if (rc != T3D_OK) return rc;
+  return t3d_x3_step_head(a, params, planes_fwd, planes_dgrad, plane_stride, table, n_entries, n_blocks, hyper, sched, static_cast<hipStream_t>(stream));
+}
+
 static const t3d_rider_set* query_set() {
   static const t3d_rider_set q = []() { t3d_rider_set r{}; r.n_ops = 1; r.n_wg = 1; r.sync = reinterpret_cast<unsigned*>(16); return r; }();
   return &q;
diff --git a/transferable3d_amd/engine.py b/transferable3d_amd/engine.py
--- a/transferable3d_amd/engine.py
+++ b/transferable3d_amd/engine.py
@@ -86,9 +86,9 @@
         self.calls.append((name, lambda s, fn=fn, ref=ref: fn(ref, s), args))
         self.lanes.append(self._lane)
 
-    def add_raw(self, name, thunk, *keep):
+    def add_raw(self, name, thunk, *keep, arg=None):
         self.keep.extend(keep)
-        self.calls.append((name, thunk, None))
+        self.calls.append((name, thunk, arg))
         self.lanes.append(self._lane)
 
     def mark(self, tag):
diff --git a/transferable3d_amd/nets.py b/transferable3d_amd/nets.py
--- a/transferable3d_amd/nets.py
+++ b/transferable3d_amd/nets.py
@@ -63,7 +63,7 @@
         def thunk(s):
             return lib.t3d_reduce_slabs(fptr(ws.buf), fptr(vs.grads),
                                         C.cast(C.c_void_p(ws.table.data_ptr() + i0 * stride), C.POINTER(abi.SlabDesc)), i1 - i0, mx, s)
-        plan.add_raw('t3d_reduce_slabs', thunk)
+        plan.add_raw('t3d_reduce_slabs', thunk, arg={'i0': i0, 'i1': i1, 'max_numel': mx})
 
     def emit_cast_weights(self, plan):
         vs, lib = self.vars, self.rt.lib
@@ -78,7 +78,7 @@
                     pf, pd = vs.x3_frag_planes
                     return lib.t3d_split_x3_frag(fptr(vs.params), C.c_void_p(pf.data_ptr()), C.c_void_p(pd.data_ptr()), vs.x3_frag_stride,
                                                  C.c_void_p(t.data_ptr()), n, nblk, s)
-                plan.add_raw('t3d_split_x3_frag', thunk)
+                plan.add_raw('t3d_split_x3_frag', thunk, arg={'vars': vs})
             return
         p16 = vs.enable_bf16()
         plan.add_raw('t3d_cast_bf16', lambda s: lib.t3d_cast_bf16(fptr(vs.params), C.c_void_p(p16.data_ptr()), vs.used, s))
@@ -127,7 +127,8 @@
 
     def emit_schedule(self, plan, sched):
         lib, hyper = self.rt.lib, self.hyper
-        plan.add_raw('t3d_schedule_step', lambda s: lib.t3d_schedule_step(fptr(hyper), C.byref(sched), s), sched)
+        plan.add_raw('t3d_schedule_step', lambda s: lib.t3d_schedule_step(fptr(hyper), C.byref(sched), s), sched,
+                     arg={'hyper': hyper, 'sched': sched})
 
     def emit_dropout_masks(self, plan, seed=1234):
         lib, hyper = self.rt.lib, self.hyper
@@ -144,7 +145,8 @@
             plan.add_raw('t3d_adam_tf_step',
                          lambda s, off=off, n=n: lib.t3d_adam_tf_step(
                              fptr(vs.params[off:]), fptr(vs.grads[off:]), fptr(vs.adam_m[off:]), fptr(vs.adam_v[off:]),
-                             n, fptr(hyper), beta1, beta2, eps, grad_scale, s))
+                             n, fptr(hyper), beta1, beta2, eps, grad_scale, s),
+                         arg={'off': off, 'n': n, 'beta1': beta1, 'beta2': beta2, 'eps': eps, 'grad_scale': grad_scale})
         self._emit_optimizer(plan, prefixes, adam)
 
     def emit_momentum(self, plan, prefixes=None, momentum=0.9, grad_scale=1.0):
diff --git a/transferable3d_amd/step.py b/transferable3d_amd/step.py
--- a/transferable3d_amd/step.py
+++ b/transferable3d_amd/step.py
@@ -1,8 +1,11 @@
+import ctypes as C
 import os
 
+import numpy as np
 import torch
 
 from . import abi
+from .abi import fptr
 from .engine import Plan
 
 
@@ -11,8 +14,12 @@
 
 class TrainStep:
     def __init__(self, engine, pre, fwd, bwd=None, opt=None, process_group=None, use_hip_graph=None, force_dist=False,
-                 one_graph=None):
+                 one_graph=None, fuse_head_tail=None):
         self.e, self.rt = engine, engine.rt
+        if fuse_head_tail is None:
+            fuse_head_tail = os.environ.get('T3D_FUSE_HEAD_TAIL', '1') != '0'
+        self.fuse_head_tail = bool(fuse_head_tail)
+        self.fused = []
         self.pre, self.fwd, self.bwd, self.opt = pre, fwd, bwd, opt
         self.train = bwd is not None
         self.pg = process_group
@@ -61,6 +68,8 @@
             calls.append((Plan.JOIN, lambda s: 0, None))
             lanes.append(0)
             two = two or p.two_streams
+        if self.fuse_head_tail:
+            calls, lanes = self._fuse_head_tail(calls, lanes)
         if self.dist and not any(c[0] == Plan.BUCKET for c in calls):
             k = next((i for i, c in enumerate(calls) if c[0] in OPTIMIZER_CALLS), len(calls))
             calls[k:k] = [(Plan.BUCKET, lambda s: 0, 0), (Plan.WAIT, lambda s: 0, 0)]
@@ -101,6 +110,63 @@
                     merged.lanes.extend(x.lanes)
             prog = prog[:k] + [t for t in tail if t[0] == 'wait'] + [('run', merged)]
         return prog
+
+    def _fuse_head_tail(self, calls, lanes):
+        lib, e = self.rt.lib, self.e
+        self.fused = []
+        real = [i for i, c in enumerate(calls) if not c[0].startswith('__') or c[0] in (Plan.BUCKET, Plan.WAIT, Plan.FLUSH)]
+        names = [calls[i][0] for i in real]
+        drop = set()
+
+        def adjacent(*want):
+            for k in range(len(names) - len(want) + 1):
+                if tuple(names[k:k + len(want)]) == want:
+                    idx = real[k:k + len(want)]
+                    if all(calls[i][2] is not None for i in idx) and not any(lanes[i] for i in idx):
+                        return idx
+            return None
+
+        idx = adjacent('t3d_schedule_step', 't3d_split_x3_frag', 't3d_pointmlp_fwd')
+        if idx is not None and self.on_gpu and hasattr(lib, 't3d_step_head') and self.rt.arith == abi.ARITH_BF16X3 and \
+                names.count('t3d_schedule_step') == 1:
+            sc, vs, a = calls[idx[0]][2], calls[idx[1]][2]['vars'], calls[idx[2]][2]
+            if lib.t3d_step_head_takes(C.byref(a)) == 1 and getattr(vs, 'x3_frag_entries', None):
+                hyper, sched = sc['hyper'], sc['sched']
+
+                def head(s, a=a, vs=vs, hyper=hyper, sched=sched):
+                    t, n, nblk = vs.frag_table()
+                    pf, pd = vs.x3_frag_planes
+                    return lib.t3d_step_head(C.byref(a), fptr(vs.params), C.c_void_p(pf.data_ptr()), C.c_void_p(pd.data_ptr()),
+                                             vs.x3_frag_stride, C.c_void_p(t.data_ptr()), n, nblk, fptr(hyper), C.byref(sched), s)
+                calls[idx[0]] = ('t3d_step_head', head, None)
+                drop.update(idx[1:])
+                self.fused.append('t3d_step_head')
+        idx = adjacent('t3d_reduce_slabs', 't3d_adam_tf_step')
+        vs = e.vars
+        if idx is not None and self.on_gpu and hasattr(lib, 't3d_reduce_slabs_adam') and not self.dist and e.dt == abi.F32 and \
+                names.count('t3d_adam_tf_step') == 1 and idx[1] == real[-1] and getattr(e, 'trained_prefixes', None) is None:
+            rd, ad = calls[idx[0]][2], calls[idx[1]][2]
+            if (ad['off'], ad['n']) == (0, vs.used) and e.finalized:
+                ws = e.ws
+                ent = ws.entries[rd['i0']:rd['i1']]
+                ranges, nblk = abi.adam_range_table(vs.used, [(go, ne) for _, go, ne, _ in ent])
+                host = (abi.AdamRange * max(len(ranges), 1))()
+                for i, (off, n, blk0) in enumerate(ranges):
+                    host[i] = abi.AdamRange(off, n, blk0, 0)
+                table = torch.as_tensor(np.frombuffer(bytes(host), dtype=np.uint8).copy()).to(self.rt.device)
+                stride = C.sizeof(abi.SlabDesc)
+
+                def tail(s, rd=rd, ad=ad, table=table, n_ranges=len(ranges), nblk=nblk):
+                    return lib.t3d_reduce_slabs_adam(
+                        fptr(ws.buf), fptr(vs.grads), C.cast(C.c_void_p(ws.table.data_ptr() + rd['i0'] * stride), C.POINTER(abi.SlabDesc)),
+                        rd['i1'] - rd['i0'], rd['max_numel'], fptr(vs.params), fptr(vs.adam_m), fptr(vs.adam_v),
+                        C.cast(C.c_void_p(table.data_ptr()), C.POINTER(abi.AdamRange)), n_ranges, nblk, fptr(e.hyper),
+                        ad['beta1'], ad['beta2'], ad['eps'], ad['grad_scale'], s)
+                calls[idx[0]] = ('t3d_reduce_slabs_adam', tail, None)
+                drop.add(idx[1])
+                self.fused.append('t3d_reduce_slabs_adam')
+        keep = [i for i in range(len(calls)) if i not in drop]
+        return [calls[i] for i in keep], [lanes[i] for i in keep]
 
     def _overlap(self, calls, lanes):
         from . import schedule
@@ -310,7 +376,7 @@
 
 def build_training_step(rt, workload, B, N, C, world=1, rank=0, process_group=None, force_dist=False, flat_allreduce=False,
                         use_hip_graph=None, inline_dropout=True, dropout_seed=1234, seed=0, state_dict=None, c=None, dtype='f32',
-                        one_graph=None):
+                        one_graph=None, fuse_head_tail=None):
     from .nets import BoxPCModel, Graph, SemiModelA, SemiModelF, make_schedule
     assert workload in WORKLOADS
     g = Graph(B, N, C, rt=rt, seed=seed, dtype=dtype)
@@ -341,7 +407,7 @@
     g.emit_adam(g.opt, prefixes=prefixes, grad_scale=1.0 / world)
     g.finalize()
     step = TrainStep(g, g.pre, g.fwd, g.bwd, g.opt, process_group=process_group, use_hip_graph=use_hip_graph,
-                     force_dist=force_dist, one_graph=one_graph)
+                     force_dist=force_dist, one_graph=one_graph, fuse_head_tail=fuse_head_tail)
     return g, model, step, loss
 
 
```

Result: faster. 27810 (median of 6 runs) (+1.3%).
